# jcyk/gtos

Hardware: AMD Instinct MI355X
Metric: graphs/sec training step (100-node AMR, batch 64) (higher is better)
Workload: dtype bf16

## Files before the change

### gtos_amd/_lib.py

```python
import ctypes
import os
import threading

import torch

_HERE = os.path.dirname(os.path.abspath(__file__))
LIB_PATH = os.path.join(_HERE, "csrc", "libgtos_hip.so")
ABI_VERSION = 25

c_p, c_i, c_l, c_f, c_u64 = ctypes.c_void_p, ctypes.c_int, ctypes.c_int64, ctypes.c_float, ctypes.c_uint64

SIGNATURES = {
    "gtos_abi_version": [],
    "gtos_pathtrie_dev_workspace": [c_l, c_l, c_p],
    "gtos_pathtrie_dev_phase_a": [c_i, c_l, c_p, c_p, c_p, c_p, c_p, c_p, c_p, ctypes.c_size_t, c_p],
    "gtos_pathtrie_dev_phase_b": [c_l, c_l, c_i, c_i, c_i, c_i, c_p, c_p, c_p, c_p, c_p, ctypes.c_size_t, c_p],
    "gtos_relbatch_dev_workspace": [c_l, c_p],
    "gtos_relbatch_dev_phase_a": [c_p, c_p, c_p, ctypes.c_size_t, c_p],
    "gtos_relbatch_dev_phase_b": [c_p, c_l, c_p, c_p, ctypes.c_size_t, c_p],
    "gtos_relbatch_dev_all_count": [c_p, c_p, c_p, ctypes.c_size_t, c_p],
    "gtos_relbatch_dev_all_keys": [c_p, c_p, c_p, ctypes.c_size_t, c_p],
    "gtos_relbatch_dev_all_fill": [c_p, c_l, c_p, c_p, ctypes.c_size_t, c_p],
    "gtos_relindex_dev_workspace": [c_l, c_p],
    "gtos_relindex_dev_phase_a": [c_p, c_p, c_p, ctypes.c_size_t, c_p],
    "gtos_relindex_dev_phase_b": [c_p, c_l, c_p, c_p, ctypes.c_size_t, c_p],
    "gtos_gemm": [c_i, c_i, c_i, c_i, c_i, c_i, c_i, c_p, c_l, c_p, c_l, c_p, c_l, c_p, c_i, c_f, c_u64, c_i, c_i, c_p, c_l, c_p],
    "gtos_rel_attn_fwd": [c_i] * 7 + [c_p, c_l, c_p, c_l, c_p, c_l, c_p, c_p, c_p, c_p, c_f, c_f, c_u64, c_p, c_l, c_p, c_p, c_p],
    "gtos_rel_attn_bwd": [c_i] * 7 + [c_p, c_l, c_p, c_l, c_p, c_l, c_p, c_p, c_p, c_p, c_p, c_f, c_f, c_u64,
                                      c_p, c_l, c_p, c_p, c_p, c_l, c_p, c_p, c_l, c_p, c_l, c_p, c_l, c_p, c_l, c_p, c_p, c_p],
    "gtos_rel_attn_bwd_bank": [c_i] * 5 + [c_p, c_l, c_p, c_l, c_p, c_p, c_p, c_p, c_p, c_p, c_p, c_p, c_i, c_p, c_l, c_p, c_p],
    "gtos_ln_residual_fwd": [c_i, c_i, c_i, c_p, c_p, c_f, c_u64, c_p, c_p, c_f, c_p, c_p, c_p, c_p],
    "gtos_ln_residual_bwd": [c_i, c_i, c_i, c_p, c_p, c_p, c_f, c_u64, c_p, c_p, c_p, c_p, c_p, c_p, c_p, c_p],
    "gtos_ln_residual_fwd2": [c_i, c_i, c_i, c_i, c_i, c_p, c_p, c_f, c_u64, c_p, c_p, c_f, c_p, c_p, c_p, c_p, c_p],
    "gtos_ln_residual_bwd2": [c_i, c_i, c_i, c_i, c_i, c_p, c_p, c_p, c_p, c_f, c_u64, c_p, c_p, c_p, c_p, c_p, c_p, c_p, c_p],
    "gtos_relu_dropout_bwd": [c_i, c_l, c_p, c_p, c_f, c_p],
    "gtos_colsum": [c_i, c_i, c_i, c_l, c_p, c_p, c_p],
    "gtos_gru_cell_fwd": [c_i, c_i, c_i, c_p, c_p, c_p, c_p, c_l, c_p, c_p, c_f, c_u64, c_l, c_p],
    "gtos_gru_step_fwd": [c_i, c_i, c_p, c_l, c_i, c_p, c_p, c_p, c_p, c_p, c_p, c_p, c_p, c_p, c_p, c_p, c_p, c_i, c_p, c_l, c_p, c_p, c_p, c_l,
                          c_f, c_u64, c_l, c_p],
    "gtos_gru_step_bwd": [c_i, c_i, c_p, c_i, c_p, c_p, c_p, c_p, c_p, c_l, c_p, c_i, c_l, c_p, c_f, c_u64, c_l, c_p, c_i, c_p, c_p, c_p, c_i, c_p],
    "gtos_gru_step_bwd_fused": [c_i, c_i, c_p, c_i, c_p, c_p, c_p, c_p, c_p, c_l, c_p, c_i, c_l, c_p, c_f, c_u64, c_l, c_p, c_i, c_p, c_p, c_p, c_i,
                                c_p, c_p, c_l, c_i, c_i, c_f, c_u64, c_l, c_p],
    "gtos_gru_weight_grads": [c_i, c_i, c_i, c_i, c_p, c_p, c_l, c_p, c_l, c_p, c_l, c_p, c_l, c_p, c_l, c_p],
    "gtos_gemm_tn_batch": [c_i, c_p, c_p, c_p, c_p, c_p, c_p, c_p, c_p, c_p, c_p, c_p],
    "gtos_embed_packed_paths": [c_i, c_i, c_i, c_l, c_p, c_p, c_p, c_p, c_i, c_i, c_p, c_f, c_u64, c_p, c_i, c_p, c_p],
    "gtos_segment_sum_rows": [c_i, c_p, c_p, c_p, c_p, c_p, c_p, c_p, c_l, c_i, c_p, c_p, c_l, c_p, c_p, c_p],
    "gtos_segment_sum_stream": [c_i, c_i, c_p, c_p, c_p, c_p, c_p, c_p, c_i, c_p, c_l, c_i, c_p, c_l, c_p, c_p],
    "gtos_segment_sum_finish": [c_i, c_p, c_p, c_i, c_p, c_l, c_p],
    "gtos_segment_sum_ranges": [c_i, c_p, c_p, c_l, c_i, c_p, c_l, c_p],
    "gtos_gru_cell_bwd": [c_i, c_i, c_i, c_p, c_p, c_p, c_l, c_p, c_p, c_p, c_f, c_u64, c_l, c_p, c_i, c_p],
    "gtos_relation_gather_mean": [c_i, c_l, c_i, c_i, c_p, c_p, c_i, c_p, c_p],
    "gtos_embed_rows_fwd": [c_i, c_l, c_i, c_i, c_p, c_p, c_p, c_f, c_u64, c_p],
    "gtos_embed_rows_bwd": [c_i, c_l, c_i, c_i, c_i, c_p, c_p, c_p, c_f, c_u64, c_p, c_l, c_p],
    "gtos_copy_nll_fwd": [c_i, c_i, c_i, c_i, c_i, c_p, c_l, c_p, c_p, c_p, c_p, c_l, c_p, c_p, c_p, c_p],
    "gtos_copy_nll_bwd": [c_i, c_i, c_i, c_i, c_i, c_p, c_l, c_p, c_p, c_p, c_p, c_l, c_p, c_p, c_p, c_p, c_p, c_p, c_p],
    "gtos_copy_ll_fwd": [c_i, c_i, c_i, c_i, c_i, c_i, c_p, c_l, c_p, c_p, c_p, c_p, c_p],
    "gtos_copy_nll_ls_prep": [c_i, c_i, c_i, c_p, c_p, c_l, c_p],
    "gtos_copy_nll_ls_fwd": [c_i] * 5 + [c_p, c_l, c_p, c_p, c_p, c_l, c_f, c_p, c_l, c_p, c_p, c_p, c_p],
    "gtos_copy_nll_ls_bwd": [c_i] * 5 + [c_p, c_l, c_p, c_p, c_p, c_l, c_f, c_p, c_l, c_p, c_p, c_p, c_p, c_p, c_p, c_p],
    "gtos_copy_eval_fwd": [c_i, c_i, c_i, c_i, c_i, c_p, c_l, c_p, c_p, c_p, c_p, c_l, c_p, c_p, c_p, c_p],
    "gtos_eval_accumulate": [c_i, c_i, c_p, c_p, c_p, c_l, c_p, c_p, c_p, c_p, c_p],
    "gtos_beam_topk": [c_i, c_i, c_i, c_p, c_l, c_p, c_p, c_p],
    "gtos_beam_advance": [c_i] * 7 + [c_p] * 13,
    "gtos_beam_reorder": [c_i, c_p, c_p, c_l, c_i, c_i, c_i, c_i, c_p, c_p, c_p, c_p, c_i, c_i, c_p, c_p, c_p, c_p, c_i, c_l, c_p, c_p,
                          c_p, c_p],
    "gtos_sample_step": [c_i] * 7 + [c_f, c_i, c_f, c_u64, c_p, c_l] + [c_p] * 11 + [c_i, c_l] + [c_p] * 4,
    "gtos_highway_fwd": [c_i, c_l, c_i, c_p, c_p, c_p, c_p],
    "gtos_highway_bwd": [c_i, c_l, c_i, c_p, c_p, c_p, c_p, c_p, c_p],
    "gtos_max_relu_fwd": [c_i, c_l, c_i, c_i, c_p, c_p, c_p, c_p],
    "gtos_max_relu_bwd": [c_i, c_l, c_i, c_i, c_p, c_p, c_p, c_p, c_p],
    "gtos_token_row_fwd": [c_i, c_l, c_i, c_i, c_i, c_p, c_p, c_p, c_p, c_f, c_u64, c_p],
    "gtos_token_row_bwd": [c_i, c_l, c_i, c_i, c_i, c_p, c_p, c_p, c_p, c_f, c_u64, c_p],
    "gtos_sqnorm": [c_l, c_p, c_p, c_p],
    "gtos_adam_step": [c_l, c_p, c_p, c_p, c_p, c_f, c_f, c_f, c_f, c_f, c_f, c_p, c_f, c_p, c_p],
    "gtos_cast_f32_to_bf16": [c_l, c_p, c_p, c_p],
    "gtos_transpose_batch_bf16": [c_i, c_p, c_p, c_i, c_p, c_p, c_p],
    "gtos_step_control": [c_i, c_p, c_p, c_p, c_i, c_i, c_p, c_p],
    "gtos_set_seed_epoch": [c_p],
    "gtos_adam_step_ctl": [c_l, c_p, c_p, c_p, c_p, c_p, c_f, c_f, c_f, c_f, c_f, c_p, c_f, c_p, c_p],
}

_lib = None
_load_lock = threading.Lock()


class GtosHipError(RuntimeError):
    pass


def load():
    global _lib
    if _lib is not None:
        return _lib
    with _load_lock:
        if _lib is not None:
            return _lib
        if not os.path.exists(LIB_PATH):
            raise GtosHipError("%s is missing: run `python -m gtos_amd.build` (or __graft_entry__.build()); "
                               "there is no CPU fallback for the gtos hot path" % LIB_PATH)
        lib = ctypes.CDLL(LIB_PATH)
        for name, args in SIGNATURES.items():
            fn = getattr(lib, name)
            fn.argtypes = args
            fn.restype = ctypes.c_int
        if lib.gtos_abi_version() != ABI_VERSION:
            raise GtosHipError("libgtos_hip.so ABI %d != binding ABI %d: rebuild" % (lib.gtos_abi_version(), ABI_VERSION))
        _lib = lib
    return _lib


def call(name, *args):
    rc = getattr(load(), name)(*args)
    if rc != 0:
        raise GtosHipError("%s failed with code %d (%s)" % (
            name, rc, "HIP launch error" if rc > 0 else "unsupported argument/shape"))


def ptr(t):
    return None if t is None else t.data_ptr()


_raw_stream = None


def stream():
    global _raw_stream
    if _raw_stream:
        return _raw_stream(torch.cuda.current_device())
    pub = torch.cuda.current_stream().cuda_stream
    if _raw_stream is None:
        try:
            raw = torch._C._cuda_getCurrentRawStream
            ok = raw(torch.cuda.current_device()) == pub
            probe = torch.cuda.Stream()
            with torch.cuda.stream(probe):
                ok = ok and raw(torch.cuda.current_device()) == probe.cuda_stream == torch.cuda.current_stream().cuda_stream
            ok = ok and raw(torch.cuda.current_device()) == pub
            _raw_stream = raw if ok else False
        except Exception:
            _raw_stream = False
    return pub


def dt(t):
    if t.dtype == torch.float32:
        return 0
    if t.dtype == torch.bfloat16:
        return 1
    raise GtosHipError("unsupported dtype %s" % t.dtype)


def require_cuda(*ts):
    for t in ts:
        if t is not None and not t.is_cuda:
            raise GtosHipError("gtos_amd ops run on the GPU only (got a %s tensor); there is no CPU fallback" % t.device)
```

### gtos_amd/csrc/gru_step.hip

```cpp
#include <cstdlib>
#include "common.h"

__attribute__((visibility("hidden"))) const void* gtos_zero_block();

#define GTOS_VMCNT(n) __builtin_amdgcn_s_waitcnt(0x0F70 | ((n) & 15) | (((n) >> 4) << 14))
#ifndef GTOS_RACE_DEMO
#define GTOS_VMCNT_LDS(n) __builtin_amdgcn_s_waitcnt(0x0070 | ((n) & 15) | (((n) >> 4) << 14))
#define GTOS_LGKM0() __builtin_amdgcn_s_waitcnt(0xc07f)
#else
#define GTOS_VMCNT_LDS(n) GTOS_VMCNT(n)
#define GTOS_LGKM0()
#endif

namespace {

constexpr int ROWB = 128, BK = 64, TM = 128, TC = 64, WROWS = 3 * TC;
constexpr int A_BYTES = TM * ROWB, B_BYTES = WROWS * ROWB;

__device__ __forceinline__ int swz(int row) { return ((row >> 1) & 7) ^ ((row >> 4) & 3); }
__device__ __forceinline__ int lds_off(int r, int c) { return r * ROWB + ((c ^ swz(r)) << 4); }

struct StepArgs {
    const bf16_t* x; int64_t ldx; int in_dim; const bf16_t* w_ih; const float* b_ih;
    const bf16_t* xg;
    const bf16_t* gf; const int* gf_idx; const bf16_t* gb; const int* gb_idx;
    const bf16_t* h_in; const int* h_idx; const bf16_t* w_hh; const float* b_hh;
    bf16_t* h_out; int n_out; bf16_t* h_fin; bf16_t* gates; bf16_t* y; int64_t ldy;
    int64_t ld_fin; const int* fin_idx;
    float p_drop; uint64_t seed; int64_t drop_base;
    int rows, hs; const void* zeros;
};

__device__ __forceinline__ void dma_rows(const bf16_t* __restrict__ base, const U128* __restrict__ zeros, int64_t ld, int rows_total,
                                         int row0, int k0, int kend, char* tile, int wave, int lane,
                                         const int* __restrict__ gather = nullptr) {
#pragma unroll
    for (int it = 0; it < TM / 32; ++it) {
        const int blk = it * 4 + wave, rl = blk * 8 + (lane >> 3);
        const int c = (lane & 7) ^ swz(rl);
        const int r = row0 + rl, k = k0 + c * 8;
        const bool ok = r < rows_total && k + 8 <= kend;
        const int64_t sr = (gather && ok) ? gather[r] : r;
        const void* src = ok ? static_cast<const void*>(base + sr * ld + k) : static_cast<const void*>(zeros);
        __builtin_amdgcn_global_load_lds((const __attribute__((address_space(1))) void*)src,
                                         (__attribute__((address_space(3))) void*)(tile + blk * 1024), 16, 0, 0);
    }
}

__device__ __forceinline__ void dma_weights(const bf16_t* __restrict__ w, const U128* __restrict__ zeros, int64_t ld, int hs,
                                            int c0, int k0, int kend, char* tile, int wave, int lane) {
#pragma unroll
    for (int it = 0; it < WROWS / 32; ++it) {
        const int blk = it * 4 + wave, rl = blk * 8 + (lane >> 3);
        const int g = rl >> 6, nt = (rl >> 4) & 3, q = (rl >> 2) & 3, e = rl & 3;
        const int wrow = g * hs + c0 + q * 16 + nt * 4 + e;
        const int c = (lane & 7) ^ swz(rl);
        const int k = k0 + c * 8;
        const bool ok = k + 8 <= kend;
        const void* src = ok ? static_cast<const void*>(w + (int64_t)wrow * ld + k) : static_cast<const void*>(zeros);
        __builtin_amdgcn_global_load_lds((const __attribute__((address_space(1))) void*)src,
                                         (__attribute__((address_space(3))) void*)(tile + blk * 1024), 16, 0, 0);
    }
}

struct RowSrc { const char* p[TM / 32]; int c[TM / 32]; };
__device__ __forceinline__ RowSrc row_src(const bf16_t* __restrict__ base, int64_t ld, int rows_total, int row0, int wave, int lane,
                                          const int* __restrict__ gather = nullptr, int zero_row = -1) {
    RowSrc s;
#pragma unroll
    for (int it = 0; it < TM / 32; ++it) {
        const int rl = (it * 4 + wave) * 8 + (lane >> 3);
        const int r = row0 + rl;
        s.c[it] = (lane & 7) ^ swz(rl);
        const bool ok = r < rows_total;
        const int64_t sr = (gather && ok) ? gather[r] : r;
        s.p[it] = (ok && sr != zero_row) ? reinterpret_cast<const char*>(base + sr * ld + s.c[it] * 8) : nullptr;
    }
    return s;
}
__device__ __forceinline__ void dma_rows_at(const RowSrc& s, const U128* __restrict__ zeros, int k0, int kend, char* tile, int wave) {
#pragma unroll
    for (int it = 0; it < TM / 32; ++it) {
        const bool ok = s.p[it] != nullptr && k0 + s.c[it] * 8 + 8 <= kend;
        const void* src = ok ? static_cast<const void*>(s.p[it] + (int64_t)k0 * 2) : static_cast<const void*>(zeros);
        __builtin_amdgcn_global_load_lds((const __attribute__((address_space(1))) void*)src,
                                         (__attribute__((address_space(3))) void*)(tile + (it * 4 + wave) * 1024), 16, 0, 0);
    }
}
__device__ __forceinline__ void dma_rows_at_z(const RowSrc& s, int k0, char* tile, int wave, int lane) {
#pragma unroll
    for (int it = 0; it < TM / 32; ++it) {
        char* blk = tile + (it * 4 + wave) * 1024;
        if (s.p[it] != nullptr)
            __builtin_amdgcn_global_load_lds((const __attribute__((address_space(1))) void*)(s.p[it] + (int64_t)k0 * 2),
                                             (__attribute__((address_space(3))) void*)blk, 16, 0, 0);
        else
            *reinterpret_cast<uint4*>(blk + lane * 16) = make_uint4(0, 0, 0, 0);
    }
}
struct WSrc { uint32_t off[WROWS / 32]; int c[WROWS / 32]; };
__device__ __forceinline__ WSrc w_src(int64_t ld, int hs, int c0, int wave, int lane) {
    WSrc s;
#pragma unroll
    for (int it = 0; it < WROWS / 32; ++it) {
        const int rl = (it * 4 + wave) * 8 + (lane >> 3);
        const int g = rl >> 6, nt = (rl >> 4) & 3, q = (rl >> 2) & 3, e = rl & 3;
        const int wrow = g * hs + c0 + q * 16 + nt * 4 + e;
        s.c[it] = (lane & 7) ^ swz(rl);
        s.off[it] = (uint32_t)(wrow * (int)ld + s.c[it] * 8) * 2u;
    }
    return s;
}
__device__ __forceinline__ void dma_weights_at(const WSrc& s, const bf16_t* __restrict__ w, const U128* __restrict__ zeros, int k0, int kend,
                                               char* tile, int wave) {
    const char* wk = reinterpret_cast<const char*>(w) + (int64_t)k0 * 2;
#pragma unroll
    for (int it = 0; it < WROWS / 32; ++it) {
        const bool ok = k0 + s.c[it] * 8 + 8 <= kend;
        const void* src = ok ? static_cast<const void*>(wk + s.off[it]) : static_cast<const void*>(zeros);
        __builtin_amdgcn_global_load_lds((const __attribute__((address_space(1))) void*)src,
                                         (__attribute__((address_space(3))) void*)(tile + (it * 4 + wave) * 1024), 16, 0, 0);
    }
}

template <int NG, int G2>
__device__ __forceinline__ void mma_tile(const char* As, const char* Bs, int wrow0, int fr, int fq, f32x4_t (&acc)[2][NG * 4]) {
#pragma unroll
    for (int ks = 0; ks < 2; ++ks) {
        bf16x8_t fa[2];
#pragma unroll
        for (int mt = 0; mt < 2; ++mt) fa[mt] = *reinterpret_cast<const bf16x8_t*>(As + lds_off(wrow0 + mt * 16 + fr, ks * 4 + fq));
#pragma unroll
        for (int g = 0; g < 3; ++g) {
            const int ag = g < 2 ? g : G2;
#pragma unroll
            for (int nt = 0; nt < 4; ++nt) {
                const bf16x8_t fb = *reinterpret_cast<const bf16x8_t*>(Bs + lds_off(g * 64 + nt * 16 + fr, ks * 4 + fq));
#pragma unroll
                for (int mt = 0; mt < 2; ++mt)
                    acc[mt][ag * 4 + nt] = __builtin_amdgcn_mfma_f32_16x16x32_bf16(fb, fa[mt], acc[mt][ag * 4 + nt], 0, 0, 0);
            }
        }
    }
}

__device__ __forceinline__ void ld16(const bf16_t* p, float (&v)[16]) {
    const uint4 a = *reinterpret_cast<const uint4*>(p), b = *reinterpret_cast<const uint4*>(p + 8);
    v[0] = lo_bf(a.x); v[1] = hi_bf(a.x); v[2] = lo_bf(a.y); v[3] = hi_bf(a.y);
    v[4] = lo_bf(a.z); v[5] = hi_bf(a.z); v[6] = lo_bf(a.w); v[7] = hi_bf(a.w);
    v[8] = lo_bf(b.x); v[9] = hi_bf(b.x); v[10] = lo_bf(b.y); v[11] = hi_bf(b.y);
    v[12] = lo_bf(b.z); v[13] = hi_bf(b.z); v[14] = lo_bf(b.w); v[15] = hi_bf(b.w);
}
__device__ __forceinline__ void st16(bf16_t* p, const float (&v)[16]) {
    *reinterpret_cast<uint4*>(p) = make_uint4(pack_bf(v[0], v[1]), pack_bf(v[2], v[3]), pack_bf(v[4], v[5]), pack_bf(v[6], v[7]));
    *reinterpret_cast<uint4*>(p + 8) = make_uint4(pack_bf(v[8], v[9]), pack_bf(v[10], v[11]), pack_bf(v[12], v[13]), pack_bf(v[14], v[15]));
}
__device__ __forceinline__ void ldf16(const float* p, float (&v)[16]) {
#pragma unroll
    for (int i = 0; i < 4; ++i) {
        const float4 a = *reinterpret_cast<const float4*>(p + i * 4);
        v[i * 4] = a.x; v[i * 4 + 1] = a.y; v[i * 4 + 2] = a.z; v[i * 4 + 3] = a.w;
    }
}

__device__ __forceinline__ float fast_tanh(float x) {
    const float e = __expf(2.f * x);
    return 1.f - 2.f * __builtin_amdgcn_rcpf(e + 1.f);
}

template <int MODE>
__device__ __forceinline__ void step_cell(const StepArgs& a, f32x4_t (&acc)[2][(MODE == 1 ? 4 : 3) * 4], int m0, int c0, int wave, int fr, int fq) {
    constexpr bool HAS_X = MODE == 1;
    constexpr int GH = HAS_X ? 3 : 2;
    const int cb = c0 + fq * 16, hs = a.hs;
    float bhr[16], bhz[16], bhn[16];
    ldf16(a.b_hh + cb, bhr); ldf16(a.b_hh + hs + cb, bhz); ldf16(a.b_hh + 2 * hs + cb, bhn);
    if constexpr (MODE != 0) {
        float t[16];
        ldf16(a.b_ih + cb, t);
#pragma unroll
        for (int i = 0; i < 16; ++i) bhr[i] += t[i];
        ldf16(a.b_ih + hs + cb, t);
#pragma unroll
        for (int i = 0; i < 16; ++i) bhz[i] += t[i];
    }
    const float ks = a.p_drop > 0.f ? 1.f / (1.f - a.p_drop) : 1.f;
#pragma unroll
    for (int mt = 0; mt < 2; ++mt) {
        const int m = m0 + wave * 32 + mt * 16 + fr;
        if (m >= a.rows) continue;
        float xr[16], xz[16], xn[16], hp[16];
        if constexpr (HAS_X) {
            ldf16(a.b_ih + 2 * hs + cb, xn);
#pragma unroll
            for (int i = 0; i < 16; ++i) { xr[i] = 0.f; xz[i] = 0.f; xn[i] += acc[mt][8 + (i >> 2)][i & 3]; }
        } else if constexpr (MODE == 2) {
            const bf16_t* fp = a.gf + (int64_t)a.gf_idx[m] * 3 * hs + cb;
            const bf16_t* bp = a.gb + (int64_t)a.gb_idx[m] * 3 * hs + cb;
            float t[16];
            ld16(fp, xr); ld16(bp, t);
#pragma unroll
            for (int i = 0; i < 16; ++i) xr[i] += t[i];
            ld16(fp + hs, xz); ld16(bp + hs, t);
#pragma unroll
            for (int i = 0; i < 16; ++i) xz[i] += t[i];
            ld16(fp + 2 * hs, xn); ld16(bp + 2 * hs, t);
#pragma unroll
            for (int i = 0; i < 16; ++i) xn[i] += t[i];
            ldf16(a.b_ih + 2 * hs + cb, t);
#pragma unroll
            for (int i = 0; i < 16; ++i) xn[i] += t[i];
        } else {
            const bf16_t* xp = a.xg + (int64_t)m * 3 * hs + cb;
            ld16(xp, xr); ld16(xp + hs, xz); ld16(xp + 2 * hs, xn);
        }
        ld16(a.h_in + (int64_t)(a.h_idx ? a.h_idx[m] : m) * hs + cb, hp);
        float gr[16], gz[16], gn[16], hn[16], o[16];
#pragma unroll
        for (int i = 0; i < 16; ++i) {
            gr[i] = 1.f / (1.f + __expf(-(xr[i] + acc[mt][(i >> 2)][i & 3] + bhr[i])));
            gz[i] = 1.f / (1.f + __expf(-(xz[i] + acc[mt][4 + (i >> 2)][i & 3] + bhz[i])));
            hn[i] = acc[mt][GH * 4 + (i >> 2)][i & 3] + bhn[i];
            hn[i] = bf2f(f2bf(hn[i]));
            gn[i] = fast_tanh(xn[i] + gr[i] * hn[i]);
            o[i] = (1.f - gz[i]) * gn[i] + gz[i] * hp[i];
        }
        bf16_t* gp = a.gates + (int64_t)m * 4 * hs + cb;
        st16(gp, gr); st16(gp + hs, gz); st16(gp + 2 * hs, gn);
        st16(gp + 3 * hs, hn);
        bf16_t* hdst = m < a.n_out ? a.h_out + (int64_t)m * hs + cb
                                   : a.h_fin + (int64_t)(a.fin_idx ? a.fin_idx[m] : m) * a.ld_fin + cb;
        st16(hdst, o);
        if (a.y) {
            if (a.p_drop > 0.f) {
#pragma unroll
                for (int i = 0; i < 16; ++i)
                    o[i] = drop_keep(a.seed, (uint64_t)(a.drop_base + (int64_t)m * a.ldy + cb + i), a.p_drop) ? o[i] * ks : 0.f;
            }
            st16(a.y + (int64_t)m * a.ldy + cb, o);
        }
    }
}

template <int MODE>
__global__ __launch_bounds__(256, 2) void gru_step_fwd_kernel(StepArgs a) {
    if (a.p_drop > 0.f) a.seed = live_seed(a.seed);
    constexpr bool HAS_X = MODE == 1;
    constexpr int NG = HAS_X ? 4 : 3;
    constexpr int GH = HAS_X ? 3 : 2;
    __shared__ __attribute__((aligned(16))) char lds[A_BYTES + B_BYTES];
    char* As = lds;
    char* Bs = lds + A_BYTES;
    const int lane = threadIdx.x & 63, wave = __builtin_amdgcn_readfirstlane(threadIdx.x >> 6);
    const int fr = lane & 15, fq = lane >> 4;
    const int nC = a.hs / TC;
    const int xcd = blockIdx.x & 7, sq = blockIdx.x >> 3;
    const int m0 = ((sq / nC) * 8 + xcd) * TM, c0 = (sq % nC) * TC;
    if (m0 >= a.rows) return;
    const U128* Z = static_cast<const U128*>(a.zeros);

    f32x4_t acc[2][NG * 4];
#pragma unroll
    for (int i = 0; i < 2; ++i)
#pragma unroll
        for (int j = 0; j < NG * 4; ++j) acc[i][j] = f32x4_t{0.f, 0.f, 0.f, 0.f};

    if constexpr (HAS_X) {
        const RowSrc xs = row_src(a.x, a.ldx, a.rows, m0, wave, lane);
        const WSrc ws = w_src(a.in_dim, a.hs, c0, wave, lane);
        for (int k0 = 0; k0 < a.in_dim; k0 += BK) {
            dma_rows_at(xs, Z, k0, a.in_dim, As, wave);
            dma_weights_at(ws, a.w_ih, Z, k0, a.in_dim, Bs, wave);
            __syncthreads();
            mma_tile<NG, 2>(As, Bs, wave * 32, fr, fq, acc);
            __syncthreads();
        }
    }
    {
        const RowSrc hsrc = row_src(a.h_in, a.hs, a.rows, m0, wave, lane, a.h_idx);
        const WSrc ws = w_src(a.hs, a.hs, c0, wave, lane);
        for (int k0 = 0; k0 < a.hs; k0 += BK) {
            dma_rows_at(hsrc, Z, k0, a.hs, As, wave);
            dma_weights_at(ws, a.w_hh, Z, k0, a.hs, Bs, wave);
            __syncthreads();
            mma_tile<NG, GH>(As, Bs, wave * 32, fr, fq, acc);
            __syncthreads();
        }
    }

    step_cell<MODE>(a, acc, m0, c0, wave, fr, fq);
}


__global__ __launch_bounds__(512, 2) void gru_step_fwd_a2w3_kernel(StepArgs a) {
    constexpr int TMW = 256, AW = TMW * ROWB;
    if (a.p_drop > 0.f) a.seed = live_seed(a.seed);
    __shared__ __attribute__((aligned(16))) char sa0[AW];
    __shared__ __attribute__((aligned(16))) char sa1[AW];
    __shared__ __attribute__((aligned(16))) char sw0[B_BYTES];
    __shared__ __attribute__((aligned(16))) char sw1[B_BYTES];
    __shared__ __attribute__((aligned(16))) char sa2[AW];
    const int lane = threadIdx.x & 63, wave = __builtin_amdgcn_readfirstlane(threadIdx.x >> 6);
    const int fr = lane & 15, fq = lane >> 4;
    const int hs = a.hs, nC = hs / TC;
    const int xcd = blockIdx.x & 7, sq = blockIdx.x >> 3;
    const int m0 = ((sq / nC) * 8 + xcd) * TMW, c0 = (sq % nC) * TC;
    if (m0 >= a.rows) return;
    const int nkx = a.in_dim / BK, nk = nkx + hs / BK;
    uint32_t axo[4], aho[4], bxo[3], bho[3];
#pragma unroll
    for (int i = 0; i < 4; ++i) {
        const int rl = (i * 8 + wave) * 8 + (lane >> 3);
        const int r = min(m0 + rl, a.rows - 1) - m0;
        const uint32_t c = (uint32_t)(((lane & 7) ^ swz(rl)) << 4);
        axo[i] = (uint32_t)r * (uint32_t)(a.ldx * 2) + c;
        aho[i] = (uint32_t)r * (uint32_t)(hs * 2) + c;
    }
#pragma unroll
    for (int i = 0; i < 3; ++i) {
        const int rl = (i * 8 + wave) * 8 + (lane >> 3);
        const int g = rl >> 6, nt = (rl >> 4) & 3, q = (rl >> 2) & 3, e = rl & 3;
        const int wrow = g * hs + c0 + q * 16 + nt * 4 + e;
        const uint32_t c = (uint32_t)(((lane & 7) ^ swz(rl)) << 4);
        bxo[i] = (uint32_t)wrow * (uint32_t)(a.in_dim * 2) + c;
        bho[i] = (uint32_t)wrow * (uint32_t)(hs * 2) + c;
    }
    const char* Xb = reinterpret_cast<const char*>(a.x + (int64_t)m0 * a.ldx);
    const char* Hb = reinterpret_cast<const char*>(a.h_in + (int64_t)m0 * hs);
    const char* Wi = reinterpret_cast<const char*>(a.w_ih);
    const char* Wh = reinterpret_cast<const char*>(a.w_hh);

    f32x4_t acc[2][16];
#pragma unroll
    for (int i = 0; i < 2; ++i)
#pragma unroll
        for (int j = 0; j < 16; ++j) acc[i][j] = f32x4_t{0.f, 0.f, 0.f, 0.f};

#define GTOS_DMA1(src, dst)                                                                                                   \
    __builtin_amdgcn_global_load_lds((const __attribute__((address_space(1))) void*)(src),                                    \
                                     (__attribute__((address_space(3))) void*)(dst), 16, 0, 0)
#define GTOS_A2W3_DMA_A(slot, s_)                                                                                             \
    {                                                                                                                         \
        const int st_ = min((s_), nk - 1);                                                                                    \
        const bool px_ = st_ < nkx;                                                                                           \
        const char* ab_ = px_ ? Xb + st_ * ROWB : Hb + (st_ - nkx) * ROWB;                                                    \
        GTOS_DMA1(ab_ + (px_ ? axo[0] : aho[0]), (slot) + (0 * 8 + wave) * 1024);                                             \
        GTOS_DMA1(ab_ + (px_ ? axo[1] : aho[1]), (slot) + (1 * 8 + wave) * 1024);                                             \
        GTOS_DMA1(ab_ + (px_ ? axo[2] : aho[2]), (slot) + (2 * 8 + wave) * 1024);                                             \
        GTOS_DMA1(ab_ + (px_ ? axo[3] : aho[3]), (slot) + (3 * 8 + wave) * 1024);                                             \
    }
#define GTOS_A2W3_DMA_W(slot, s_)                                                                                             \
    {                                                                                                                         \
        const int st_ = min((s_), nk - 1);                                                                                    \
        const bool px_ = st_ < nkx;                                                                                           \
        const char* bb_ = px_ ? Wi + st_ * ROWB : Wh + (st_ - nkx) * ROWB;                                                    \
        GTOS_DMA1(bb_ + (px_ ? bxo[0] : bho[0]), (slot) + (0 * 8 + wave) * 1024);                                             \
        GTOS_DMA1(bb_ + (px_ ? bxo[1] : bho[1]), (slot) + (1 * 8 + wave) * 1024);                                             \
        GTOS_DMA1(bb_ + (px_ ? bxo[2] : bho[2]), (slot) + (2 * 8 + wave) * 1024);                                             \
    }
#define GTOS_A2W3_STEP(sa_, sw_, sa_n, sw_n, s_)                                                                              \
    {                                                                                                                         \
        GTOS_VMCNT_LDS(4);                                  \
        __builtin_amdgcn_s_barrier();                       \
        GTOS_A2W3_DMA_W(sw_n, (s_) + 1);                                                                                      \
        GTOS_A2W3_DMA_A(sa_n, (s_) + 2);                                                                                      \
        {                                                                                                                     \
            _Pragma("unroll") for (int ks = 0; ks < 2; ++ks) {                                                                \
                bf16x8_t fa[2], fb[12];                                                                                       \
                _Pragma("unroll") for (int mt = 0; mt < 2; ++mt)                                                              \
                    fa[mt] = *reinterpret_cast<const bf16x8_t*>((sa_) + lds_off(wave * 32 + mt * 16 + fr, ks * 4 + fq));      \
                _Pragma("unroll") for (int t = 0; t < 12; ++t)                                                                \
                    fb[t] = *reinterpret_cast<const bf16x8_t*>((sw_) + lds_off(t * 16 + fr, ks * 4 + fq));                    \
                _Pragma("unroll") for (int g = 0; g < 2; ++g)                                                                 \
                    _Pragma("unroll") for (int nt = 0; nt < 4; ++nt)                                                          \
                        _Pragma("unroll") for (int mt = 0; mt < 2; ++mt)                                                      \
                            acc[mt][g * 4 + nt] = __builtin_amdgcn_mfma_f32_16x16x32_bf16(fb[g * 4 + nt], fa[mt], acc[mt][g * 4 + nt], 0, 0, 0); \
                if ((s_) < nkx) {                                                                                             \
                    _Pragma("unroll") for (int nt = 0; nt < 4; ++nt)                                                          \
                        _Pragma("unroll") for (int mt = 0; mt < 2; ++mt)                                                      \
                            acc[mt][8 + nt] = __builtin_amdgcn_mfma_f32_16x16x32_bf16(fb[8 + nt], fa[mt], acc[mt][8 + nt], 0, 0, 0); \
                } else {                                                                                                      \
                    _Pragma("unroll") for (int nt = 0; nt < 4; ++nt)                                                          \
                        _Pragma("unroll") for (int mt = 0; mt < 2; ++mt)                                                      \
                            acc[mt][12 + nt] = __builtin_amdgcn_mfma_f32_16x16x32_bf16(fb[8 + nt], fa[mt], acc[mt][12 + nt], 0, 0, 0); \
                }                                                                                                             \
            }                                                                                                                 \
        }                                                                                                                     \
    }

    if (nk > 0) {
        GTOS_A2W3_DMA_A(sa0, 0);
        GTOS_A2W3_DMA_W(sw0, 0);
        GTOS_A2W3_DMA_A(sa1, 1);
    }
    for (int s = 0; s + 6 <= nk; s += 6) {
        GTOS_A2W3_STEP(sa0, sw0, sa2, sw1, s);
        GTOS_A2W3_STEP(sa1, sw1, sa0, sw0, s + 1);
        GTOS_A2W3_STEP(sa2, sw0, sa1, sw1, s + 2);
        GTOS_A2W3_STEP(sa0, sw1, sa2, sw0, s + 3);
        GTOS_A2W3_STEP(sa1, sw0, sa0, sw1, s + 4);
        GTOS_A2W3_STEP(sa2, sw1, sa1, sw0, s + 5);
    }
    GTOS_VMCNT(0);
#undef GTOS_A2W3_STEP
#undef GTOS_A2W3_DMA_W
#undef GTOS_A2W3_DMA_A
#undef GTOS_DMA1
    step_cell<1>(a, acc, m0, c0, wave, fr, fq);
}


struct Raw16 { uint4 a, b; };
__device__ __forceinline__ void unpack16(const Raw16& r, float (&v)[16]) {
    v[0] = lo_bf(r.a.x); v[1] = hi_bf(r.a.x); v[2] = lo_bf(r.a.y); v[3] = hi_bf(r.a.y);
    v[4] = lo_bf(r.a.z); v[5] = hi_bf(r.a.z); v[6] = lo_bf(r.a.w); v[7] = hi_bf(r.a.w);
    v[8] = lo_bf(r.b.x); v[9] = hi_bf(r.b.x); v[10] = lo_bf(r.b.y); v[11] = hi_bf(r.b.y);
    v[12] = lo_bf(r.b.z); v[13] = hi_bf(r.b.z); v[14] = lo_bf(r.b.w); v[15] = hi_bf(r.b.w);
}
__device__ __forceinline__ Raw16 ldraw16(const bf16_t* p) {
    Raw16 r;
    r.a = *reinterpret_cast<const uint4*>(p);
    r.b = *reinterpret_cast<const uint4*>(p + 8);
    return r;
}

constexpr int P_ROWS = 32;
constexpr int P_TM = 4 * P_ROWS;

template <int KT>
__global__ __launch_bounds__(256, 1) void gru_l1_fwd_persistent_kernel(StepArgs a, int n_workers) {
    extern __shared__ __attribute__((aligned(16))) char plds[];
    constexpr int HS = 64 * KT;
    constexpr int A_TILE = P_ROWS * ROWB;
    const int lane = threadIdx.x & 63, wave = __builtin_amdgcn_readfirstlane(threadIdx.x >> 6);
    const int fr = lane & 15, fq = lane >> 4;
    char* Ws = plds;
    char* Aw = plds + KT * B_BYTES + wave * (KT * A_TILE);
    const int nC = KT;
    const int xcd = blockIdx.x & 7, sub = blockIdx.x >> 3;
    const int ct = sub % nC, worker = (sub / nC) * 8 + xcd, c0 = ct * TC;
    const U128* Z = static_cast<const U128*>(a.zeros);
#pragma unroll
    for (int kt = 0; kt < KT; ++kt) dma_weights(a.w_hh, Z, HS, HS, c0, kt * BK, HS, Ws + kt * B_BYTES, wave, lane);
    __syncthreads();

    const int cb = c0 + fq * 16;
    float bhr[16], bhz[16], bhn[16], bin[16];
    {
        float t[16];
        ldf16(a.b_hh + cb, bhr); ldf16(a.b_ih + cb, t);
#pragma unroll
        for (int i = 0; i < 16; ++i) bhr[i] += t[i];
        ldf16(a.b_hh + HS + cb, bhz); ldf16(a.b_ih + HS + cb, t);
#pragma unroll
        for (int i = 0; i < 16; ++i) bhz[i] += t[i];
        ldf16(a.b_hh + 2 * HS + cb, bhn); ldf16(a.b_ih + 2 * HS + cb, bin);
    }
    const int n_tiles = (a.rows + P_TM - 1) / P_TM;

    auto dma_A = [&](int tile) {
        const int r0 = tile * P_TM + wave * P_ROWS;
#pragma unroll
        for (int kt = 0; kt < KT; ++kt)
#pragma unroll
            for (int it = 0; it < P_ROWS / 8; ++it) {
                const int rl = it * 8 + (lane >> 3);
                const int c = (lane & 7) ^ swz(rl);
                const int r = r0 + rl;
                const void* src = r < a.rows ? static_cast<const void*>(a.h_in + (int64_t)r * HS + kt * BK + c * 8)
                                             : static_cast<const void*>(Z);
                __builtin_amdgcn_global_load_lds((const __attribute__((address_space(1))) void*)src,
                                                 (__attribute__((address_space(3))) void*)(Aw + kt * A_TILE + it * 1024), 16, 0, 0);
            }
    };
    struct Pre { Raw16 f[3], b[3], h; };
    auto gather = [&](int tile, Pre (&P)[2]) {
#pragma unroll
        for (int mt = 0; mt < 2; ++mt) {
            int m = tile * P_TM + wave * P_ROWS + mt * 16 + fr;
            m = m < a.rows ? m : a.rows - 1;
            const bf16_t* fp = a.gf + (int64_t)a.gf_idx[m] * 3 * HS + cb;
            const bf16_t* bp = a.gb + (int64_t)a.gb_idx[m] * 3 * HS + cb;
#pragma unroll
            for (int g = 0; g < 3; ++g) { P[mt].f[g] = ldraw16(fp + g * HS); P[mt].b[g] = ldraw16(bp + g * HS); }
            P[mt].h = ldraw16(a.h_in + (int64_t)m * HS + cb);
        }
    };

    int tile = worker;
    Pre P[2];
    if (tile < n_tiles) { dma_A(tile); gather(tile, P); }
    for (; tile < n_tiles; tile += n_workers) {
        f32x4_t acc[2][12];
#pragma unroll
        for (int i = 0; i < 2; ++i)
#pragma unroll
            for (int j = 0; j < 12; ++j) acc[i][j] = f32x4_t{0.f, 0.f, 0.f, 0.f};
#pragma unroll
        for (int kt = 0; kt < KT; ++kt) {
            const char* As = Aw + kt * A_TILE;
            const char* Bs = Ws + kt * B_BYTES;
#pragma unroll
            for (int ks = 0; ks < 2; ++ks) {
                bf16x8_t fa[2];
#pragma unroll
                for (int mt = 0; mt < 2; ++mt) fa[mt] = *reinterpret_cast<const bf16x8_t*>(As + lds_off(mt * 16 + fr, ks * 4 + fq));
#pragma unroll
                for (int g = 0; g < 3; ++g)
#pragma unroll
                    for (int nt = 0; nt < 4; ++nt) {
                        const bf16x8_t fb = *reinterpret_cast<const bf16x8_t*>(Bs + lds_off(g * 64 + nt * 16 + fr, ks * 4 + fq));
#pragma unroll
                        for (int mt = 0; mt < 2; ++mt)
                            acc[mt][g * 4 + nt] = __builtin_amdgcn_mfma_f32_16x16x32_bf16(fb, fa[mt], acc[mt][g * 4 + nt], 0, 0, 0);
                    }
            }
        }
        __builtin_amdgcn_s_waitcnt(0xc07f);
        const int next = tile + n_workers;
        if (next < n_tiles) dma_A(next);
#pragma unroll
        for (int mt = 0; mt < 2; ++mt) {
            const int m = tile * P_TM + wave * P_ROWS + mt * 16 + fr;
            float xr[16], xz[16], xn[16], hp[16], t[16];
            unpack16(P[mt].f[0], xr); unpack16(P[mt].b[0], t);
#pragma unroll
            for (int i = 0; i < 16; ++i) xr[i] += t[i];
            unpack16(P[mt].f[1], xz); unpack16(P[mt].b[1], t);
#pragma unroll
            for (int i = 0; i < 16; ++i) xz[i] += t[i];
            unpack16(P[mt].f[2], xn); unpack16(P[mt].b[2], t);
#pragma unroll
            for (int i = 0; i < 16; ++i) xn[i] += t[i] + bin[i];
            unpack16(P[mt].h, hp);
            float gr[16], gz[16], gn[16], hn[16], o[16];
#pragma unroll
            for (int i = 0; i < 16; ++i) {
                gr[i] = 1.f / (1.f + __expf(-(xr[i] + acc[mt][(i >> 2)][i & 3] + bhr[i])));
                gz[i] = 1.f / (1.f + __expf(-(xz[i] + acc[mt][4 + (i >> 2)][i & 3] + bhz[i])));
                hn[i] = bf2f(f2bf(acc[mt][8 + (i >> 2)][i & 3] + bhn[i]));
                gn[i] = fast_tanh(xn[i] + gr[i] * hn[i]);
                o[i] = (1.f - gz[i]) * gn[i] + gz[i] * hp[i];
            }
            if (m < a.rows) {
                bf16_t* gp = a.gates + (int64_t)m * 4 * HS + cb;
                st16(gp, gr); st16(gp + HS, gz); st16(gp + 2 * HS, gn);
                st16(gp + 3 * HS, hn);
                bf16_t* hdst = m < a.n_out ? a.h_out + (int64_t)m * HS + cb
                                           : a.h_fin + (int64_t)(a.fin_idx ? a.fin_idx[m] : m) * a.ld_fin + cb;
                st16(hdst, o);
            }
        }
        if (next < n_tiles) gather(next, P);
    }
}


struct StepBwdArgs {
    const bf16_t* d4_prev; int rows_prev; const bf16_t* wh_t;
    const bf16_t* gates; const bf16_t* hprev; const int* hprev_idx; const bf16_t* dy; int64_t ldy;
    void* dh; int dh_bf16; int64_t ld_dh; bf16_t* d4; float* bias_part; int n_partials;
    bf16_t* hp_out;
    const int* sum_idx;
    const void* dh_src;
    int zero_row;
    float p_drop; uint64_t seed; int64_t drop_base;
    int rows, hs; const void* zeros;
    const bf16_t* wi_t; bf16_t* dinp; int64_t ld_dinp; int n_in; int dinp_acc;
    float p_in; uint64_t seed_in; int64_t in_drop_base;
};

#define GTOS_DPP(v, ctrl) __builtin_bit_cast(float, __builtin_amdgcn_update_dpp(0, __builtin_bit_cast(int, (v)), (ctrl), 0xF, 0xF, true))
__device__ __forceinline__ float row16_sum(float v) {
    v += GTOS_DPP(v, 0xB1); v += GTOS_DPP(v, 0x4E); v += GTOS_DPP(v, 0x141); v += GTOS_DPP(v, 0x140);
    return v;
}

__device__ __forceinline__ void dma_wt(const bf16_t* __restrict__ w, int64_t ld, int c0, int k0, char* tile, int wave, int lane) {
#pragma unroll
    for (int it = 0; it < TC / 32; ++it) {
        const int blk = it * 4 + wave, rl = blk * 8 + (lane >> 3);
        const int nt = (rl >> 4) & 3, q = (rl >> 2) & 3, e = rl & 3;
        const int wrow = c0 + q * 16 + nt * 4 + e;
        const int c = (lane & 7) ^ swz(rl);
        const void* src = static_cast<const void*>(w + (int64_t)wrow * ld + k0 + c * 8);
        __builtin_amdgcn_global_load_lds((const __attribute__((address_space(1))) void*)src,
                                         (__attribute__((address_space(3))) void*)(tile + blk * 1024), 16, 0, 0);
    }
}

template <int NB, bool SKIP>
__device__ __forceinline__ void kloop_a2(const bf16_t* __restrict__ A, int64_t lda, int rows_total, int m0, const bf16_t* __restrict__ W,
                                         int64_t ldw, int n0, int nsub, int hs, const U128* __restrict__ Z, char* a0, char* a1, char* ws,
                                         f32x4_t (&acc)[2][NB * 4], int wave, int lane) {
    const int fr = lane & 15, fq = lane >> 4, nst = 3 * hs / BK;
#define GTOS_KA_A(slot, s_)                                                                                                   \
    {                                                                                                                         \
        const int kk_ = min((s_), nst - 1) * BK, ak_ = SKIP ? (kk_ < 2 * hs ? kk_ : kk_ + hs) : kk_;                            \
        dma_rows(A, Z, lda, rows_total, m0, ak_, ak_ + BK, (slot), wave, lane);                                               \
    }
#define GTOS_KA_STEP(cur, nxt, s_)                                                                                            \
    {                                                                                                                         \
        _Pragma("unroll") for (int h = 0; h < NB; ++h)                                                                        \
            if (h < nsub) dma_wt(W, ldw, n0 + h * TC, (s_) * BK, ws + h * TC * ROWB, wave, lane);                             \
        GTOS_VMCNT_LDS(0);                                                                                                    \
        __builtin_amdgcn_s_barrier();                                          \
        GTOS_KA_A(nxt, (s_) + 1);                                                                                             \
        __builtin_amdgcn_sched_barrier(0);                                                                                    \
        _Pragma("unroll") for (int ks = 0; ks < 2; ++ks) {                                                                    \
            bf16x8_t fa[2], fb[4];                                                                                            \
            _Pragma("unroll") for (int mt = 0; mt < 2; ++mt)                                                                  \
                fa[mt] = *reinterpret_cast<const bf16x8_t*>((cur) + lds_off(wave * 32 + mt * 16 + fr, ks * 4 + fq));          \
            _Pragma("unroll") for (int h = 0; h < NB; ++h) {                                                                  \
                if (h < nsub) {                                                                                               \
                    _Pragma("unroll") for (int nt = 0; nt < 4; ++nt)                                                          \
                        fb[nt] = *reinterpret_cast<const bf16x8_t*>(ws + h * TC * ROWB + lds_off(nt * 16 + fr, ks * 4 + fq)); \
                    _Pragma("unroll") for (int mt = 0; mt < 2; ++mt)                                                          \
                        _Pragma("unroll") for (int nt = 0; nt < 4; ++nt)                                                      \
                            acc[mt][h * 4 + nt] = __builtin_amdgcn_mfma_f32_16x16x32_bf16(fb[nt], fa[mt], acc[mt][h * 4 + nt], 0, 0, 0); \
                }                                                                                                             \
            }                                                                                                                 \
        }                                                                                                                     \
        GTOS_LGKM0();                                       \
        __builtin_amdgcn_s_barrier();                               \
    }
    GTOS_KA_A(a0, 0);
    int s = 0;
    for (; s + 2 <= nst; s += 2) {
        GTOS_KA_STEP(a0, a1, s);
        GTOS_KA_STEP(a1, a0, s + 1);
    }
    if (s < nst) GTOS_KA_STEP(a0, a1, s);
    GTOS_VMCNT(0);
    __builtin_amdgcn_s_barrier();
#undef GTOS_KA_STEP
#undef GTOS_KA_A
}

template <int NS>
__device__ __forceinline__ void dinp_tile(const StepBwdArgs& a, int m0, int n0, char* As, char* Bs, char* A1, int wave, int lane) {
    if (m0 >= a.rows_prev) return;
    const int fr = lane & 15, fq = lane >> 4, hs = a.hs;
    const U128* Z = static_cast<const U128*>(a.zeros);
    const int nsub = min(NS, (a.n_in - n0) / TC);
    f32x4_t acc[2][NS * 4];
#pragma unroll
    for (int i = 0; i < 2; ++i)
#pragma unroll
        for (int j = 0; j < NS * 4; ++j) acc[i][j] = f32x4_t{0.f, 0.f, 0.f, 0.f};
    kloop_a2<NS, false>(a.d4_prev, 4 * (int64_t)hs, a.rows_prev, m0, a.wi_t, 3 * (int64_t)hs, n0, nsub, hs, Z, As, A1, Bs, acc, wave, lane);
    const float ks_in = a.p_in > 0.f ? 1.f / (1.f - a.p_in) : 1.f;
    const uint64_t seed_in = a.p_in > 0.f ? live_seed(a.seed_in) : 0;
    Raw16 oldv[2][NS];
    if (a.dinp_acc) {
#pragma unroll
        for (int mt = 0; mt < 2; ++mt) {
            const int m = min(m0 + wave * 32 + mt * 16 + fr, a.rows_prev - 1);
#pragma unroll
            for (int h = 0; h < NS; ++h)
                if (h < nsub) oldv[mt][h] = ldraw16(a.dinp + (int64_t)m * a.ld_dinp + n0 + h * TC + fq * 16);
        }
    }
#pragma unroll
    for (int mt = 0; mt < 2; ++mt) {
        const int m = m0 + wave * 32 + mt * 16 + fr;
        if (m >= a.rows_prev) continue;
#pragma unroll
        for (int h = 0; h < NS; ++h) {
            if (h >= nsub) continue;
            const int nb = n0 + h * TC + fq * 16;
            float v[16];
#pragma unroll
            for (int i = 0; i < 16; ++i) v[i] = acc[mt][h * 4 + (i >> 2)][i & 3];
            if (a.p_in > 0.f) {
#pragma unroll
                for (int i = 0; i < 16; ++i)
                    v[i] = drop_keep(seed_in, (uint64_t)(a.in_drop_base + (int64_t)m * a.n_in + nb + i), a.p_in) ? v[i] * ks_in : 0.f;
            }
            bf16_t* dp = a.dinp + (int64_t)m * a.ld_dinp + nb;
            if (a.dinp_acc) {
                float old[16];
                unpack16(oldv[mt][h], old);
#pragma unroll
                for (int i = 0; i < 16; ++i) v[i] += old[i];
            }
            st16(dp, v);
        }
    }
}

template <int NS = 2>
__global__ __launch_bounds__(256, 3) void gru_step_bwd_kernel(StepBwdArgs a) {
    if (a.p_drop > 0.f) a.seed = live_seed(a.seed);
    __shared__ __attribute__((aligned(16))) char lds[A_BYTES];
    __shared__ __attribute__((aligned(16))) char lds_w[NS * TC * ROWB];
    __shared__ __attribute__((aligned(16))) char lds_a1[A_BYTES];
    __shared__ float btab[4 * TC];
    char* As = lds;
    char* Bs = lds_w;
    const int lane = threadIdx.x & 63, wave = __builtin_amdgcn_readfirstlane(threadIdx.x >> 6);
    const int fr = lane & 15, fq = lane >> 4;
    const int hs = a.hs, nC = hs / TC;
    const int nB = a.dinp ? (a.n_in + NS * TC - 1) / (NS * TC) : 0, per = nC + nB;
    const int xcd = blockIdx.x & 7, sq = blockIdx.x >> 3;
    const int m0 = ((sq / per) * 8 + xcd) * TM, role = sq % per;
    if (role >= nC) { dinp_tile<NS>(a, m0, (role - nC) * NS * TC, As, Bs, lds_a1, wave, lane); return; }
    const int c0 = role * TC;
    if (m0 >= a.rows) return;
    const U128* Z = static_cast<const U128*>(a.zeros);
    if (a.bias_part) { btab[threadIdx.x] = 0.f; }

    f32x4_t acc[2][4];
#pragma unroll
    for (int i = 0; i < 2; ++i)
#pragma unroll
        for (int j = 0; j < 4; ++j) acc[i][j] = f32x4_t{0.f, 0.f, 0.f, 0.f};

    if (a.d4_prev && a.sum_idx) {
        const RowSrc src = row_src(a.d4_prev, 4 * (int64_t)hs, a.rows, m0, wave, lane, a.sum_idx, a.zero_row);
        for (int kk = 0; kk < 3 * hs; kk += BK) {
            const int ak = kk < 2 * hs ? kk : kk + hs;
            dma_rows_at_z(src, ak, As, wave, lane);
            dma_wt(a.wh_t, 3 * (int64_t)hs, c0, kk, Bs, wave, lane);
            __syncthreads();
#pragma unroll
            for (int ks = 0; ks < 2; ++ks) {
                bf16x8_t fa[2], fb[4];
#pragma unroll
                for (int mt = 0; mt < 2; ++mt) fa[mt] = *reinterpret_cast<const bf16x8_t*>(As + lds_off(wave * 32 + mt * 16 + fr, ks * 4 + fq));
#pragma unroll
                for (int nt = 0; nt < 4; ++nt) fb[nt] = *reinterpret_cast<const bf16x8_t*>(Bs + lds_off(nt * 16 + fr, ks * 4 + fq));
#pragma unroll
                for (int mt = 0; mt < 2; ++mt)
#pragma unroll
                    for (int nt = 0; nt < 4; ++nt)
                        acc[mt][nt] = __builtin_amdgcn_mfma_f32_16x16x32_bf16(fb[nt], fa[mt], acc[mt][nt], 0, 0, 0);
            }
            __syncthreads();
        }
    } else if (a.d4_prev && m0 < a.rows_prev) {
        kloop_a2<1, true>(a.d4_prev, 4 * (int64_t)hs, a.rows_prev, m0, a.wh_t, 3 * (int64_t)hs, c0, 1, hs, Z, As, lds_a1, Bs, acc, wave, lane);
    } else if (a.bias_part) {
        __syncthreads();
    }

    const int cb = c0 + fq * 16;
    const float ks = a.p_drop > 0.f ? 1.f / (1.f - a.p_drop) : 1.f;
#pragma unroll
    for (int mt = 0; mt < 2; ++mt) {
        const int m_raw = m0 + wave * 32 + mt * 16 + fr;
        const bool valid = m_raw < a.rows;
        const int m = valid ? m_raw : a.rows - 1;
        float gr[16], gz[16], gn[16], hn[16], hp[16], g[16];
        const bf16_t* gp = a.gates + (int64_t)m * 4 * hs + cb;
        ld16(gp, gr); ld16(gp + hs, gz); ld16(gp + 2 * hs, gn);
        ld16(gp + 3 * hs, hn);
        ld16(a.hprev + (int64_t)(a.hprev_idx ? a.hprev_idx[m] : m) * hs + cb, hp);
        float* dhp = static_cast<float*>(a.dh) + (int64_t)m * a.ld_dh + cb;
        bf16_t* dhb = static_cast<bf16_t*>(a.dh) + (int64_t)m * a.ld_dh + cb;
        if (a.sum_idx) {
            const int64_t sr = a.sum_idx[m];
            if (sr == a.zero_row) {
#pragma unroll
                for (int i = 0; i < 16; ++i) g[i] = 0.f;
            } else if (a.dh_bf16) ld16(static_cast<const bf16_t*>(a.dh_src) + sr * hs + cb, g);
            else ldf16(static_cast<const float*>(a.dh_src) + sr * hs + cb, g);
        } else if (a.dh_bf16) ld16(dhb, g); else ldf16(dhp, g);
#pragma unroll
        for (int i = 0; i < 16; ++i) g[i] += acc[mt][i >> 2][i & 3];
        if (a.dy) {
            float dyv[16];
            ld16(a.dy + (int64_t)m * a.ldy + cb, dyv);
#pragma unroll
            for (int i = 0; i < 16; ++i) {
                float t2 = dyv[i];
                if (a.p_drop > 0.f) t2 = drop_keep(a.seed, (uint64_t)(a.drop_base + (int64_t)m * a.ldy + cb + i), a.p_drop) ? t2 * ks : 0.f;
                g[i] += t2;
            }
        }
        float dr_[16], dz_[16], dn_[16], dhn[16];
#pragma unroll
        for (int i = 0; i < 16; ++i) {
            const float dn = g[i] * (1.f - gz[i]);
            const float dz = g[i] * (hp[i] - gn[i]);
            dn_[i] = dn * (1.f - gn[i] * gn[i]);
            dhn[i] = dn_[i] * gr[i];
            dr_[i] = dn_[i] * hn[i] * gr[i] * (1.f - gr[i]);
            dz_[i] = dz * gz[i] * (1.f - gz[i]);
            g[i] *= gz[i];
            if (!valid) { dn_[i] = 0.f; dhn[i] = 0.f; dr_[i] = 0.f; dz_[i] = 0.f; }
        }
        if (valid) {
            if (a.dh_bf16) {
                st16(dhb, g);
            } else {
#pragma unroll
                for (int i = 0; i < 4; ++i)
                    *reinterpret_cast<float4*>(dhp + i * 4) = make_float4(g[i * 4], g[i * 4 + 1], g[i * 4 + 2], g[i * 4 + 3]);
            }
            bf16_t* dp = a.d4 + (int64_t)m * 4 * hs + cb;
            st16(dp, dr_); st16(dp + hs, dz_); st16(dp + 2 * hs, dn_); st16(dp + 3 * hs, dhn);
            if (a.hp_out) st16(a.hp_out + (int64_t)m * hs + cb, hp);
        }
        if (a.bias_part) {
#pragma unroll
            for (int i = 0; i < 16; ++i) {
                const float t0 = row16_sum(bf2f(f2bf(dr_[i]))), t1 = row16_sum(bf2f(f2bf(dz_[i])));
                const float t2 = row16_sum(bf2f(f2bf(dn_[i]))), t3 = row16_sum(bf2f(f2bf(dhn[i])));
                if (fr == 0) {
                    atomicAdd(&btab[0 * TC + fq * 16 + i], t0); atomicAdd(&btab[1 * TC + fq * 16 + i], t1);
                    atomicAdd(&btab[2 * TC + fq * 16 + i], t2); atomicAdd(&btab[3 * TC + fq * 16 + i], t3);
                }
            }
        }
    }
    if (a.bias_part) {
        __syncthreads();
        const int q = threadIdx.x >> 6, ch = threadIdx.x & 63;
        float* dst = a.bias_part + (int64_t)(blockIdx.x % a.n_partials) * 4 * hs + q * hs + c0 + ch;
        atomicAdd(dst, btab[threadIdx.x]);
    }
}


}

extern "C" int gtos_gru_step_fwd(int rows, int hs, const void* x, int64_t ldx, int in_dim, const void* w_ih, const float* b_ih,
                                 const void* xg, const void* gf, const int* gf_idx, const void* gb, const int* gb_idx,
                                 const void* h_in, const int* h_idx, const void* w_hh, const float* b_hh,
                                 void* h_out, int n_out, void* h_fin, int64_t ld_fin, const int* fin_idx, void* gates, void* y, int64_t ldy,
                                 float p_drop, uint64_t seed, int64_t drop_base, void* stream) {
    if (rows <= 0) return 0;
    if (hs <= 0 || hs % TC) return -22;
    if (!h_in || !w_hh || !b_hh || !gates) return -23;
    if ((n_out > 0 && !h_out) || (n_out < rows && !h_fin)) return -23;
    if (h_fin && (ld_fin < hs || ld_fin % 8)) return -25;
    const int mode = x ? 1 : (gf ? 2 : 0);
    if (mode == 1) {
        if (!w_ih || !b_ih || in_dim <= 0 || in_dim % 8 || ldx % 8 || (uintptr_t)x % 16 || (uintptr_t)w_ih % 16) return -24;
    } else if (mode == 2) {
        if (!gb || !gf_idx || !gb_idx || !b_ih || (uintptr_t)gf % 16 || (uintptr_t)gb % 16) return -24;
    } else if (!xg || (uintptr_t)xg % 16) return -24;
    if ((uintptr_t)h_in % 16 || (uintptr_t)w_hh % 16 || (uintptr_t)gates % 16 || (uintptr_t)h_out % 16 || (uintptr_t)h_fin % 16 ||
        (uintptr_t)b_hh % 16 || (uintptr_t)b_ih % 16) return -25;
    if (y && ((uintptr_t)y % 16 || ldy % 8)) return -25;
    StepArgs a;
    a.x = (const bf16_t*)x; a.ldx = ldx; a.in_dim = in_dim; a.w_ih = (const bf16_t*)w_ih; a.b_ih = b_ih; a.xg = (const bf16_t*)xg;
    a.gf = (const bf16_t*)gf; a.gf_idx = gf_idx; a.gb = (const bf16_t*)gb; a.gb_idx = gb_idx;
    a.h_in = (const bf16_t*)h_in; a.h_idx = h_idx; a.w_hh = (const bf16_t*)w_hh; a.b_hh = b_hh;
    a.h_out = (bf16_t*)h_out; a.n_out = n_out; a.h_fin = (bf16_t*)h_fin; a.gates = (bf16_t*)gates; a.y = (bf16_t*)y; a.ldy = ldy;
    a.ld_fin = ld_fin; a.fin_idx = fin_idx;
    a.p_drop = p_drop; a.seed = seed; a.drop_base = drop_base; a.rows = rows; a.hs = hs;
    a.zeros = gtos_zero_block();
    if (!a.zeros) return -5;
    const long long nM = (rows + TM - 1) / TM, nC = hs / TC;
    const long long nblk = ((nM + 7) / 8) * 8 * nC;
    if (nblk > 0x7fffffffLL) return -6;
    hipStream_t s = static_cast<hipStream_t>(stream);
    if (mode == 2 && hs == 256 && !h_idx && !y && rows >= 16384) {
        constexpr int KT = 4;
        const size_t lds_bytes = (size_t)KT * B_BYTES + 4 * KT * P_ROWS * ROWB;
        static bool configured = false;
        if (!configured) {
            if (hipFuncSetAttribute(reinterpret_cast<const void*>(gru_l1_fwd_persistent_kernel<KT>),
                                    hipFuncAttributeMaxDynamicSharedMemorySize, (int)lds_bytes) != hipSuccess) return -7;
            configured = true;
        }
        const int n_cu = 256, n_workers = n_cu / KT;
        hipLaunchKernelGGL(gru_l1_fwd_persistent_kernel<KT>, dim3(n_cu), dim3(256), lds_bytes, s, a, n_workers);
        GTOS_CHECK_LAUNCH();
        return 0;
    }
    static const bool use_a2w3 = !(getenv("GTOS_GRU_FWD_A2W3") && getenv("GTOS_GRU_FWD_A2W3")[0] == '0');
    if (mode == 1 && use_a2w3 && rows >= 8192 && in_dim % 64 == 0 && (in_dim / 64 + hs / 64) % 6 == 0 && !h_idx && ldx < (1 << 20) &&
        (int64_t)3 * hs * (in_dim > hs ? in_dim : hs) * 2 < (1LL << 31)) {
        const long long nM8 = (rows + 255) / 256, nblk8 = ((nM8 + 7) / 8) * 8 * nC;
        hipLaunchKernelGGL(gru_step_fwd_a2w3_kernel, dim3((unsigned)nblk8), dim3(512), 0, s, a);
    }
    else if (mode == 1) hipLaunchKernelGGL(gru_step_fwd_kernel<1>, dim3((unsigned)nblk), dim3(256), 0, s, a);
    else if (mode == 2) hipLaunchKernelGGL(gru_step_fwd_kernel<2>, dim3((unsigned)nblk), dim3(256), 0, s, a);
    else hipLaunchKernelGGL(gru_step_fwd_kernel<0>, dim3((unsigned)nblk), dim3(256), 0, s, a);
    GTOS_CHECK_LAUNCH();
    return 0;
}

extern "C" int gtos_gru_step_bwd_fused(int rows, int hs, const void* d4_prev, int rows_prev, const void* w_hh_t,
                                       const void* gates, const void* hprev, const int* hprev_idx, const void* dy, int64_t ldy,
                                       void* dh, int dh_dtype, int64_t ld_dh, void* d4, float p_drop, uint64_t seed, int64_t drop_base,
                                       float* bias_partials, int n_partials, void* hprev_out, const int* sum_idx, const void* dh_src,
                                       int zero_row,
                                       const void* w_ih_t, void* dinp, int64_t ld_dinp, int n_in, int dinp_accumulate, float p_in,
                                       uint64_t seed_in, int64_t in_drop_base, void* stream) {
    const bool role_b = dinp != nullptr && d4_prev != nullptr && rows_prev > 0;
    if (rows <= 0 && !role_b) return 0;
    if (hs <= 0 || hs % TC) return -22;
    if (rows > 0) {
        if (!gates || !hprev || !dh || !d4 || (d4_prev && !w_hh_t)) return -23;
        if (sum_idx && (!dh_src || (uintptr_t)dh_src % 16)) return -23;
    }
    if (dinp && (!d4_prev || !w_ih_t || sum_idx)) return -23;
    if (dinp && (n_in <= 0 || n_in % TC || ld_dinp < n_in || ld_dinp % 8 || (uintptr_t)dinp % 16 || (uintptr_t)w_ih_t % 16)) return -27;
    if (bias_partials && n_partials < 1) return -26;
    if ((uintptr_t)d4_prev % 16 || (uintptr_t)w_hh_t % 16 || (uintptr_t)gates % 16 || (uintptr_t)hprev % 16 || (uintptr_t)dh % 16 ||
        (uintptr_t)d4 % 16 || (dy && ((uintptr_t)dy % 16 || ldy % 8)) || (rows > 0 && (ld_dh < hs || ld_dh % 8)) ||
        (uintptr_t)hprev_out % 16) return -25;
    StepBwdArgs a;
    a.d4_prev = (const bf16_t*)d4_prev; a.rows_prev = d4_prev ? rows_prev : 0; a.wh_t = (const bf16_t*)w_hh_t;
    a.gates = (const bf16_t*)gates; a.hprev = (const bf16_t*)hprev; a.hprev_idx = hprev_idx; a.dy = (const bf16_t*)dy; a.ldy = ldy;
    a.dh = dh; a.dh_bf16 = dh_dtype == GTOS_BF16; a.ld_dh = ld_dh; a.d4 = (bf16_t*)d4; a.bias_part = bias_partials; a.n_partials = n_partials;
    a.hp_out = (bf16_t*)hprev_out; a.sum_idx = sum_idx; a.dh_src = dh_src; a.zero_row = sum_idx ? zero_row : -1;
    a.wi_t = (const bf16_t*)w_ih_t; a.dinp = role_b ? (bf16_t*)dinp : nullptr; a.ld_dinp = ld_dinp; a.n_in = n_in; a.dinp_acc = dinp_accumulate;
    a.p_in = p_in; a.seed_in = seed_in; a.in_drop_base = in_drop_base;
    a.p_drop = p_drop; a.seed = seed; a.drop_base = drop_base; a.rows = rows > 0 ? rows : 0; a.hs = hs;
    a.zeros = gtos_zero_block();
    if (!a.zeros) return -5;
    const long long cover = role_b && rows_prev > a.rows ? rows_prev : a.rows;
    const long long nM = (cover + TM - 1) / TM, per = hs / TC + (role_b ? (n_in + 2 * TC - 1) / (2 * TC) : 0);
    const long long nblk = ((nM + 7) / 8) * 8 * per;
    if (nblk > 0x7fffffffLL) return -6;
    hipLaunchKernelGGL(gru_step_bwd_kernel<2>, dim3((unsigned)nblk), dim3(256), 0, static_cast<hipStream_t>(stream), a);
    GTOS_CHECK_LAUNCH();
    return 0;
}

extern "C" int gtos_gru_step_bwd(int rows, int hs, const void* d4_prev, int rows_prev, const void* w_hh_t,
                                 const void* gates, const void* hprev, const int* hprev_idx, const void* dy, int64_t ldy, void* dh, int dh_dtype,
                                 int64_t ld_dh, void* d4, float p_drop, uint64_t seed, int64_t drop_base, float* bias_partials,
                                 int n_partials, void* hprev_out, const int* sum_idx, const void* dh_src, int zero_row, void* stream) {
    return gtos_gru_step_bwd_fused(rows, hs, d4_prev, rows_prev, w_hh_t, gates, hprev, hprev_idx, dy, ldy, dh, dh_dtype, ld_dh, d4,
                                   p_drop, seed, drop_base, bias_partials, n_partials, hprev_out, sum_idx, dh_src, zero_row,
                                   nullptr, nullptr, 0, 0, 0, 0.f, 0, 0, stream);
}

GTOS_SEED_EPOCH_SETTER(gru_step)
```

### gtos_amd/csrc/rowops.hip

```cpp
#include "common.h"

namespace {

constexpr int LN_MAXC = 2;

template <typename TX, typename TR, typename TY>
__global__ __launch_bounds__(256) void ln_fwd_kernel(int rows, int d, const TX* __restrict__ x, const TR* __restrict__ r,
                                                     float p_drop, uint64_t seed, const float* __restrict__ gamma,
                                                     const float* __restrict__ beta, float eps, TY* __restrict__ y, bf16_t* __restrict__ y2,
                                                     float* __restrict__ mean, float* __restrict__ rstd) {
    if (p_drop > 0.f) seed = live_seed(seed);
    const int lane = threadIdx.x & 63;
    const int row = blockIdx.x * 4 + (threadIdx.x >> 6);
    if (row >= rows) return;
    const float ks = p_drop > 0.f ? 1.f / (1.f - p_drop) : 1.f;
    float z[LN_MAXC][8];
    float s = 0.f;
#pragma unroll
    for (int cI = 0; cI < LN_MAXC; ++cI) {
        const int c = (cI * 64 + lane) * 8;
#pragma unroll
        for (int e = 0; e < 8; ++e) z[cI][e] = 0.f;
        if (c < d) {
            Vec8<TX>::load(x + (int64_t)row * d + c, z[cI]);
// ... 816 lines not shown
                                    void* stream) {
    return gtos_ln_residual_fwd2(dtype, dtype, dtype, rows, d, x, r, p_drop, seed, gamma, beta, eps, y, nullptr, mean, rstd, stream);
}

extern "C" int gtos_ln_residual_bwd2(int x_dtype, int r_dtype, int y_dtype, int rows, int d, const void* dy, const void* dy2_bf16,
                                     const void* x, const void* r, float p_drop, uint64_t seed, const float* gamma, const float* mean,
                                     const float* rstd, void* dx, void* dr, float* dgamma, float* dbeta, void* stream) {
    if (d % 8 || d > 512 * LN_MAXC) return -20;
    if (rows <= 0) return 0;
    if (!dy && !dy2_bf16) return -23;
    if ((uintptr_t)x % 16 || (uintptr_t)r % 16 || (uintptr_t)dy % 16 || (uintptr_t)dy2_bf16 % 16 || (uintptr_t)dx % 16 || (uintptr_t)dr % 16) return -25;
    hipStream_t s = static_cast<hipStream_t>(stream);
    int nb = (rows + 31) / 32; if (nb > 256) nb = 256; if (nb < 1) nb = 1;
    dim3 grid(nb), block(256);
#define X(dx_, dr_, dy_, TX, TR, TY)                                                                                                   \
    if (x_dtype == dx_ && r_dtype == dr_ && y_dtype == dy_) {                                                                          \
        hipLaunchKernelGGL((ln_bwd_kernel<TX, TR, TY>), grid, block, 0, s, rows, d, (const TY*)dy, (const bf16_t*)dy2_bf16,            \
                           (const TX*)x, (const TR*)r, p_drop, seed, gamma, mean, rstd, (TX*)dx, (TR*)dr, dgamma, dbeta);              \
        GTOS_CHECK_LAUNCH();                                                                                                           \
        return 0;                                                                                                                      \
    }
    GTOS_LN_COMBOS(X)
#undef X
    return -21;
}

extern "C" int gtos_ln_residual_bwd(int dtype, int rows, int d, const void* dy, const void* x, const void* r, float p_drop,
                                    uint64_t seed, const float* gamma, const float* mean, const float* rstd,
                                    void* dx, void* dr, float* dgamma, float* dbeta, void* stream) {
    return gtos_ln_residual_bwd2(dtype, dtype, dtype, rows, d, dy, nullptr, x, r, p_drop, seed, gamma, mean, rstd, dx, dr, dgamma, dbeta,
                                 stream);
}

extern "C" int gtos_relu_dropout_bwd(int dtype, int64_t n, void* dh, const void* h, float p_drop, void* stream) {
    if (n % 8) return -21;
    if (n == 0) return 0;
    hipStream_t s = static_cast<hipStream_t>(stream);
    const float ks = p_drop > 0.f ? 1.f / (1.f - p_drop) : 1.f;
    dim3 grid(grid_for(n / 8, 256)), block(256);
    if (dtype == GTOS_BF16) hipLaunchKernelGGL(relu_drop_bwd_kernel<bf16_t>, grid, block, 0, s, n / 8, (bf16_t*)dh, (const bf16_t*)h, ks);
    else hipLaunchKernelGGL(relu_drop_bwd_kernel<float>, grid, block, 0, s, n / 8, (float*)dh, (const float*)h, ks);
    GTOS_CHECK_LAUNCH();
    return 0;
}

extern "C" int gtos_colsum(int dtype, int rows, int N, int64_t ld, const void* dy, float* out, void* stream) {
    if (rows <= 0 || N <= 0) return 0;
    hipStream_t s = static_cast<hipStream_t>(stream);
    const int gx = (N + 511) / 512;
    int rpb = (rows + 1023) / 1024; if (rpb < 64) rpb = 64;
    dim3 grid(gx, (rows + rpb - 1) / rpb), block(256);
    if (dtype == GTOS_BF16) hipLaunchKernelGGL(colsum_kernel<bf16_t>, grid, block, 0, s, rows, N, ld, (const bf16_t*)dy, out, rpb);
    else hipLaunchKernelGGL(colsum_kernel<float>, grid, block, 0, s, rows, N, ld, (const float*)dy, out, rpb);
    GTOS_CHECK_LAUNCH();
    return 0;
}

extern "C" int gtos_gru_cell_fwd(int dtype, int rows, int hs, const void* xg, const void* hg, void* h, void* y, int64_t ldy,
                                 void* hprev_save, void* gates, float p_drop, uint64_t seed, int64_t drop_base, void* stream) {
    if (hs % 8) return -22;
    if (rows <= 0) return 0;
    hipStream_t s = static_cast<hipStream_t>(stream);
    dim3 grid(grid_for((int64_t)rows * hs / 8, 256)), block(256);
    if (dtype == GTOS_BF16) hipLaunchKernelGGL(gru_fwd_kernel<bf16_t>, grid, block, 0, s, rows, hs, (const bf16_t*)xg, (const bf16_t*)hg, (bf16_t*)h, (bf16_t*)y, ldy, (bf16_t*)hprev_save, (bf16_t*)gates, p_drop, seed, drop_base);
    else hipLaunchKernelGGL(gru_fwd_kernel<float>, grid, block, 0, s, rows, hs, (const float*)xg, (const float*)hg, (float*)h, (float*)y, ldy, (float*)hprev_save, (float*)gates, p_drop, seed, drop_base);
    GTOS_CHECK_LAUNCH();
    return 0;
}

extern "C" int gtos_gru_cell_bwd(int dtype, int rows, int hs, const void* gates, const void* hprev, const void* dy, int64_t ldy,
                                 float* dh, void* dxg, void* dhg, float p_drop, uint64_t seed, int64_t drop_base,
                                 float* bias_partials, int n_partials, void* stream) {
    if (hs % 8) return -22;
    if (rows <= 0) return 0;
    if (bias_partials && (256 % (hs / 8) != 0 || n_partials < 1)) return -26;
    hipStream_t s = static_cast<hipStream_t>(stream);
    int nb = grid_for((int64_t)rows * hs / 8, 256);
    if (bias_partials && nb > n_partials) nb = n_partials;
    dim3 grid(nb), block(256);
    const size_t sh = bias_partials ? (size_t)4 * hs * sizeof(float) : 0;
    if (dtype == GTOS_BF16) hipLaunchKernelGGL(gru_bwd_kernel<bf16_t>, grid, block, sh, s, rows, hs, (const bf16_t*)gates, (const bf16_t*)hprev, (const bf16_t*)dy, ldy, dh, (bf16_t*)dxg, (bf16_t*)dhg, p_drop, seed, drop_base, bias_partials);
    else hipLaunchKernelGGL(gru_bwd_kernel<float>, grid, block, sh, s, rows, hs, (const float*)gates, (const float*)hprev, (const float*)dy, ldy, dh, (float*)dxg, (float*)dhg, p_drop, seed, drop_base, bias_partials);
    GTOS_CHECK_LAUNCH();
    return 0;
}

extern "C" int gtos_relation_gather_mean(int dtype, int64_t P, int K, int d, const void* bank, const int64_t* idx, int zero_row0,
                                         void* out, void* stream) {
    if (d % 8) return -23;
    if (P <= 0) return 0;
    hipStream_t s = static_cast<hipStream_t>(stream);
    dim3 grid(grid_for(P * (d / 8), 256)), block(256);
    if (dtype == GTOS_BF16) hipLaunchKernelGGL(gather_mean_kernel<bf16_t>, grid, block, 0, s, P, K, d, (const bf16_t*)bank, idx, zero_row0, (bf16_t*)out);
    else hipLaunchKernelGGL(gather_mean_kernel<float>, grid, block, 0, s, P, K, d, (const float*)bank, idx, zero_row0, (float*)out);
    GTOS_CHECK_LAUNCH();
    return 0;
}


extern "C" int gtos_embed_rows_fwd(int dtype, int64_t n, int dim, int dim_pad, const int64_t* tok, const float* table, void* out,
                                   float p_drop, uint64_t seed, void* stream) {
    if (dim_pad % 8 || dim_pad < dim) return -24;
    if (n <= 0) return 0;
    hipStream_t s = static_cast<hipStream_t>(stream);
    dim3 grid(grid_for(n * (dim_pad / 8), 256)), block(256);
    if (dtype == GTOS_BF16) hipLaunchKernelGGL(embed_rows_fwd_kernel<bf16_t>, grid, block, 0, s, n, dim, dim_pad, tok, table, (bf16_t*)out, p_drop, seed);
    else hipLaunchKernelGGL(embed_rows_fwd_kernel<float>, grid, block, 0, s, n, dim, dim_pad, tok, table, (float*)out, p_drop, seed);
    GTOS_CHECK_LAUNCH();
    return 0;
}

extern "C" int gtos_embed_packed_paths(int dtype, int L, int R, int64_t n_rows, const int64_t* bank, const int* order, const int* offs,
                                       const float* table, int dim, int dim_pad, void* x, float p_drop, uint64_t seed, void* onehot, int vp,
                                       int64_t* tokens, void* stream) {
    if (dim_pad % 8 || dim_pad < dim || L < 1 || L > 64 || R < 1) return -24;
    if (onehot && (vp < 8 || vp % 8 || (uintptr_t)onehot % 16)) return -24;
    if (!bank || !order || !offs || !table || !x || (uintptr_t)x % 16) return -23;
    if (n_rows <= 0) return 0;
    hipStream_t s = static_cast<hipStream_t>(stream);
    dim3 grid(grid_for(n_rows * (dim_pad / 8), 256)), block(256);
    if (dtype == GTOS_BF16)
        hipLaunchKernelGGL(embed_packed_paths_kernel<bf16_t>, grid, block, 0, s, L, R, n_rows, bank, order, offs, table, dim, dim_pad, (bf16_t*)x,
                           p_drop, seed, (bf16_t*)onehot, vp, tokens);
    else
        hipLaunchKernelGGL(embed_packed_paths_kernel<float>, grid, block, 0, s, L, R, n_rows, bank, order, offs, table, dim, dim_pad, (float*)x,
                           p_drop, seed, (bf16_t*)onehot, vp, tokens);
    GTOS_CHECK_LAUNCH();
    return 0;
}

extern "C" int gtos_embed_rows_bwd(int dtype, int64_t n, int V, int dim, int dim_pad, const int64_t* tok, const void* dout,
                                   float* dtable, float p_drop, uint64_t seed, float* workspace, int64_t workspace_bytes, void* stream) {
    if (dim_pad % 8 || dim_pad < dim) return -24;
    const int use_lds = (size_t)V * dim_pad * 4 <= 60 * 1024;
    if (n <= 0) return 0;
    hipStream_t s = static_cast<hipStream_t>(stream);
    int64_t nb = (n + 511) / 512; if (nb > 2048) nb = 2048; if (nb < 1) nb = 1;
    const int64_t table_bytes = (int64_t)V * dim_pad * 4;
    float* partials = nullptr;
    if (use_lds && workspace && nb > 8) {
        if (workspace_bytes < table_bytes) return -24;
        const int64_t fit = workspace_bytes / table_bytes;
        if (nb > fit) nb = fit;
        partials = workspace;
    }
    const int64_t rpb = (n + nb - 1) / nb;
    dim3 grid((unsigned)((n + rpb - 1) / rpb)), block(256);
    const size_t sh = use_lds ? (size_t)table_bytes : 0;
#define GTOS_EMB_BWD(T, L) hipLaunchKernelGGL((embed_rows_bwd_kernel<T, L>), grid, block, sh, s, n, V, dim, dim_pad, tok, (const T*)dout, dtable, p_drop, seed, rpb, partials)
    if (dtype == GTOS_BF16) { if (use_lds) GTOS_EMB_BWD(bf16_t, true); else GTOS_EMB_BWD(bf16_t, false); }
    else { if (use_lds) GTOS_EMB_BWD(float, true); else GTOS_EMB_BWD(float, false); }
#undef GTOS_EMB_BWD
    GTOS_CHECK_LAUNCH();
    if (partials) {
        const int total = V * dim_pad;
        const int slices = grid.x >= 64 ? 16 : 1;
        hipLaunchKernelGGL(embed_reduce_kernel, dim3((total + 255) / 256, slices), dim3(256), 0, s, (int)grid.x, V, dim, dim_pad, partials, dtable);
        GTOS_CHECK_LAUNCH();
    }
    return 0;
}

extern "C" int gtos_segment_sum_rows(int n_chunks, const int* rows, const int* chunk_node, const int* chunk_start, const int* chunk_cnt,
                                     const int* chunk_slot, const void* src, const void* src2, int64_t ld_src, int width,
                                     void* dst, void* dst2, int64_t ld_dst, float* heavy, float* heavy2, void* stream) {
    if (n_chunks <= 0) return 0;
    if (width <= 0 || width % 8 || width > 1536 || ld_src % 8 || ld_dst % 8 || (uintptr_t)src % 16 || (uintptr_t)dst % 16 ||
        (uintptr_t)src2 % 16 || (uintptr_t)dst2 % 16) return -24;
    if (!chunk_node || !chunk_start || !chunk_cnt || !src || !dst || (chunk_slot && !heavy)) return -23;
    if (src2 && (!dst2 || (chunk_slot && !heavy2))) return -23;
    hipStream_t s = static_cast<hipStream_t>(stream);
    const int nblk = (n_chunks + 3) / 4;
    const dim3 grid((unsigned)(nblk < 4096 ? nblk : 4096)), block(256);
#define GTOS_SEG(S, Q) hipLaunchKernelGGL((seg_sum_kernel<S, Q>), grid, block, 0, s, n_chunks, rows, chunk_node, chunk_start, chunk_cnt, \
                                          chunk_slot, (const bf16_t*)src, (const bf16_t*)src2, ld_src, width, (bf16_t*)dst, (bf16_t*)dst2, \
                                          ld_dst, heavy, heavy2)
    if (src2) { if (width <= 512) GTOS_SEG(1, 2); else if (width <= 1024) GTOS_SEG(2, 2); else GTOS_SEG(3, 2); }
    else { if (width <= 512) GTOS_SEG(1, 1); else if (width <= 1024) GTOS_SEG(2, 1); else GTOS_SEG(3, 1); }
#undef GTOS_SEG
    GTOS_CHECK_LAUNCH();
    return 0;
}

extern "C" int gtos_segment_sum_stream(int n_chunks, int total_rows, const int* rows, const int* chunk_node, const int* chunk_start,
                                       const int* chunk_cnt, const int* chunk_slot, const int* wave_off, int n_waves, const void* src,
                                       int64_t ld_src, int width, void* dst, int64_t ld_dst, float* heavy, void* stream) {
    if (n_chunks <= 0 || n_waves <= 0) return 0;
    if (width <= 0 || width % 256 || width > 1536 || ld_src % 8 || ld_dst % 8 || (uintptr_t)src % 16 || (uintptr_t)dst % 16) return -24;
    if (!rows || !chunk_node || !chunk_start || !chunk_cnt || !wave_off || !src || !dst || (chunk_slot && !heavy) || total_rows <= 0) return -23;
    SegStreamArgs a;
    a.n_chunks = n_chunks; a.total_rows = total_rows; a.n_waves = n_waves;
    a.rows = rows; a.chunk_node = chunk_node; a.chunk_start = chunk_start; a.chunk_cnt = chunk_cnt; a.chunk_slot = chunk_slot;
    a.wave_off = wave_off; a.src = (const bf16_t*)src; a.ld_src = ld_src; a.dst = (bf16_t*)dst; a.ld_dst = ld_dst; a.heavy = heavy;
    hipStream_t s = static_cast<hipStream_t>(stream);
    const dim3 grid((unsigned)((n_waves + 3) / 4)), block(256);
#define GTOS_SEGS(S, H) hipLaunchKernelGGL((seg_sum_stream_kernel<S, H>), grid, block, 0, s, a.n_chunks, a.total_rows, a.n_waves, a.rows, \
        a.chunk_node, a.chunk_start, a.chunk_cnt, a.chunk_slot, a.wave_off, a.src, a.ld_src, a.dst, a.ld_dst, a.heavy)
    switch (width / 256) {
        case 1: GTOS_SEGS(0, true); break;
        case 2: GTOS_SEGS(1, false); break;
        case 3: GTOS_SEGS(1, true); break;
        case 4: GTOS_SEGS(2, false); break;
        case 5: GTOS_SEGS(2, true); break;
        default: GTOS_SEGS(3, false); break;
    }
#undef GTOS_SEGS
    GTOS_CHECK_LAUNCH();
    return 0;
}

extern "C" int gtos_segment_sum_finish(int n_heavy, const int* heavy_node, const float* heavy, int width, void* dst, int64_t ld_dst,
                                       void* stream) {
    if (n_heavy <= 0) return 0;
    if (width <= 0 || width % 8 || ld_dst % 8 || !heavy_node || !heavy || !dst) return -24;
    const int64_t n = (int64_t)n_heavy * (width / 8);
    hipLaunchKernelGGL(seg_finish_kernel, dim3((unsigned)((n + 255) / 256)), dim3(256), 0, static_cast<hipStream_t>(stream), n_heavy,
                       heavy_node, heavy, width, (bf16_t*)dst, ld_dst);
    GTOS_CHECK_LAUNCH();
    return 0;
}

extern "C" int gtos_segment_sum_ranges(int n_seg, const int* ranges, const void* src, int64_t ld_src, int width, void* dst, int64_t ld_dst,
                                       void* stream) {
    if (n_seg <= 0) return 0;
    if (width <= 0 || width % 8 || width > 1536 || ld_src % 8 || ld_dst % 8 || (uintptr_t)src % 16 || (uintptr_t)dst % 16) return -24;
    if (!ranges || !src || !dst) return -23;
    hipStream_t s = static_cast<hipStream_t>(stream);
    const dim3 grid((unsigned)((n_seg + 3) / 4)), block(256);
#define GTOS_SEG(S) hipLaunchKernelGGL(seg_sum_range_kernel<S>, grid, block, 0, s, n_seg, ranges, (const bf16_t*)src, ld_src, width, \
                                       (bf16_t*)dst, ld_dst)
    if (width <= 512) GTOS_SEG(1); else if (width <= 1024) GTOS_SEG(2); else GTOS_SEG(3);
#undef GTOS_SEG
    GTOS_CHECK_LAUNCH();
    return 0;
}

extern "C" int gtos_sqnorm(int64_t n, const float* g, float* out, void* stream) {
    if (n <= 0) return 0;
    hipStream_t s = static_cast<hipStream_t>(stream);
    hipLaunchKernelGGL(sqnorm_kernel, dim3(grid_for(n, 256 * 8)), dim3(256), 0, s, n, g, out);
    GTOS_CHECK_LAUNCH();
    return 0;
}

extern "C" int gtos_adam_step(int64_t n, float* p, const float* g, float* m, float* v, float lr, float beta1, float beta2,
                              float eps, float weight_decay, float gscale, const float* sqnorm, float max_norm,
                              void* bf16_mirror, void* stream) {
    if (n <= 0) return 0;
    hipStream_t s = static_cast<hipStream_t>(stream);
    hipLaunchKernelGGL(adam_kernel, dim3(grid_for(n, 256 * 4)), dim3(256), 0, s, n, p, g, m, v, lr, beta1, beta2, eps, weight_decay,
                       gscale, sqnorm, max_norm, (bf16_t*)bf16_mirror, (const float*)nullptr);
    GTOS_CHECK_LAUNCH();
    return 0;
}

extern "C" int gtos_adam_step_ctl(int64_t n, float* p, const float* g, float* m, float* v, const float* ctl, float beta1, float beta2,
                                  float eps, float weight_decay, float gscale, const float* sqnorm, float max_norm,
                                  void* bf16_mirror, void* stream) {
    if (n <= 0) return 0;
    if (!ctl) return -23;
    hipStream_t s = static_cast<hipStream_t>(stream);
    hipLaunchKernelGGL(adam_kernel, dim3(grid_for(n, 256 * 4)), dim3(256), 0, s, n, p, g, m, v, 0.f, beta1, beta2, eps, weight_decay,
                       gscale, sqnorm, max_norm, (bf16_t*)bf16_mirror, ctl);
    GTOS_CHECK_LAUNCH();
    return 0;
}

extern "C" int gtos_step_control(int phase, const float* loss, double* state, float* flag, int warmup_steps, int embed_dim,
                                 float* ctl, void* stream) {
    if ((phase != 0 && phase != 1) || !loss || !state || !flag || !ctl || warmup_steps < 1 || embed_dim < 1) return -23;
    hipLaunchKernelGGL(step_control_kernel, dim3(1), dim3(64), 0, static_cast<hipStream_t>(stream), phase, loss, state, flag,
                       (double)warmup_steps, (double)embed_dim, ctl);
    GTOS_CHECK_LAUNCH();
    return 0;
}

extern "C" int gtos_cast_f32_to_bf16(int64_t n, const float* src, void* dst, void* stream) {
    if (n <= 0) return 0;
    hipStream_t s = static_cast<hipStream_t>(stream);
    hipLaunchKernelGGL(cast_bf16_kernel, dim3(grid_for(n, 256 * 4)), dim3(256), 0, s, n, src, (bf16_t*)dst);
    GTOS_CHECK_LAUNCH();
    return 0;
}

extern "C" int gtos_transpose_batch_bf16(int n_mat, const int64_t* desc, const int* tile_start, int total_tiles, const void* src,
                                         void* dst, void* stream) {
    if (n_mat <= 0 || total_tiles <= 0) return 0;
    if (!desc || !tile_start || !src || !dst) return -23;
    hipLaunchKernelGGL(transpose_batch_kernel, dim3((unsigned)total_tiles), dim3(256), 0, static_cast<hipStream_t>(stream), n_mat, desc,
                       tile_start, (const bf16_t*)src, (bf16_t*)dst);
    GTOS_CHECK_LAUNCH();
    return 0;
}

extern "C" int gtos_set_seed_epoch(const void* epoch) {
    int rc = gtosi_gemm_set_seed_epoch(epoch);
    if (!rc) rc = gtosi_rel_attn_set_seed_epoch(epoch);
    if (!rc) rc = gtosi_rowops_set_seed_epoch(epoch);
    if (!rc) rc = gtosi_gru_step_set_seed_epoch(epoch);
    if (!rc) rc = gtosi_tokenenc_set_seed_epoch(epoch);
    return rc;
}

extern "C" int gtos_abi_version(void) { return 25; }

GTOS_SEED_EPOCH_SETTER(rowops)
```

### gtos_amd/gru.py

```python
import contextlib
import os

import torch

from . import _lib
from ._lib import call, dt, ptr, stream
from .ops import (gemm, compute_weight, next_seed, weight_t, _grad_target, _splitk, side_stream as _side_stream, side_ok, defer_side_join, _Timed,
                  embed_bwd_workspace, _workspace, WORKSPACE_BYTES, note_memory)


def _cell_fwd(A, hs, xg, hg, h, y, y_off_elems, ldy, hprev, gates, p, seed, drop_base):
    yp = None if y is None else y.data_ptr() + y_off_elems * y.element_size()
    call("gtos_gru_cell_fwd", dt(xg), A, hs, ptr(xg), ptr(hg), ptr(h), yp, ldy, ptr(hprev), ptr(gates),
         float(p), seed, drop_base, stream())


N_BIAS_PARTIALS = 1024

FUSE = "x"
SIDE_STREAM = os.environ.get("GTOS_GRU_SIDE", "1") != "0"
SIDE_MIN_ROWS = 200000


def _step_fwd(A, hs, x, xg, h_in, wi, b_ih, wh, b_hh, h_out, n_out, h_fin, gates, y, y_off_elems, ldy, p, seed, drop_base,
              h_idx=None, gf=None, gf_idx=None, gb=None, gb_idx=None, fin_idx=None, tag=None):
    yp = None if y is None else y.data_ptr() + y_off_elems * y.element_size()
    need_bi = x is not None or gf is not None
    name = tag or "gru_step_fwd_%s" % ("x" if x is not None else ("tables" if gf is not None else "xg"))
    units = A if tag is None else A * 2 * (x.shape[1] + hs + 4 * hs + hs + (hs if y is not None else 0))
    with _Timed(name, detail=True, units=units):
        _step_fwd_call(A, hs, x, xg, h_in, wi, b_ih, wh, b_hh, h_out, n_out, h_fin, gates, yp, ldy, p, seed, drop_base,
                       h_idx, gf, gf_idx, gb, gb_idx, need_bi, fin_idx)


def _step_fwd_call(A, hs, x, xg, h_in, wi, b_ih, wh, b_hh, h_out, n_out, h_fin, gates, yp, ldy, p, seed, drop_base,
                   h_idx, gf, gf_idx, gb, gb_idx, need_bi, fin_idx=None):
    call("gtos_gru_step_fwd", A, hs, ptr(x), 0 if x is None else x.stride(0), 0 if x is None else x.shape[1],
         ptr(wi) if x is not None else None, ptr(b_ih) if need_bi else None, ptr(xg),
         ptr(gf), ptr(gf_idx), ptr(gb), ptr(gb_idx), ptr(h_in), ptr(h_idx), ptr(wh), ptr(b_hh),
         ptr(h_out), n_out, ptr(h_fin), hs if h_fin is None else h_fin.stride(0), ptr(fin_idx), ptr(gates), yp, ldy,
         float(p), seed, drop_base, stream())


def _step_bwd(A, hs, d4_prev, rows_prev, wh_t, gates, hprev, dy_ptr, ldy, dh, d4, p, seed, drop_base, bpart, hprev_idx=None, hp_out=None,
              sum_idx=None, dh_src=None, zero_row=-1):
    with _Timed("gru_step_bwd_%s" % ("trie" if hprev_idx is not None else "rows"), detail=True, units=A):
        call("gtos_gru_step_bwd", A, hs, ptr(d4_prev), rows_prev if d4_prev is not None else 0, ptr(wh_t), ptr(gates), ptr(hprev),
             ptr(hprev_idx), dy_ptr, ldy, ptr(dh), dt(dh), dh.stride(0), ptr(d4), float(p), seed, drop_base,
             ptr(bpart), N_BIAS_PARTIALS if bpart is not None else 0, ptr(hp_out), ptr(sum_idx), ptr(dh_src), int(zero_row), stream())


def _cell_bwd(A, hs, gates, hprev, dy, dy_off_elems, ldy, dh, dxg, dhg, p, seed, drop_base, bpart):
    dyp = None if dy is None else dy.data_ptr() + dy_off_elems * dy.element_size()
    call("gtos_gru_cell_bwd", dt(gates), A, hs, ptr(gates), ptr(hprev), dyp, ldy, ptr(dh), ptr(dxg), ptr(dhg),
         float(p), seed, drop_base, ptr(bpart), 0 if bpart is None else bpart.shape[0], stream())


class BiGRUFinalFn(torch.autograd.Function):

    @staticmethod
    def forward(ctx, x, batch_sizes, hs, num_layers, p_drop, *weights):
        L, R = len(batch_sizes), batch_sizes[0]
        offs = [0]
        for a in batch_sizes:
            offs.append(offs[-1] + a)
        N = offs[-1]
        assert x.shape[0] == N
        dev, dtp = x.device, x.dtype
        inp = x.contiguous()
        saved = []
        finals = None
        for l in range(num_layers):
            last = l == num_layers - 1
            Y = None if last else torch.empty((N, 2 * hs), dtype=dtp, device=dev)
            seed = next_seed() if (p_drop > 0 and not last) else 0
            pl = p_drop if not last else 0.0
            finals = []
            layer_saved = []
            for direction in (0, 1):
                w_ih, w_hh, b_ih, b_hh = weights[l * 8 + direction * 4: l * 8 + direction * 4 + 4]
                wi, wh = compute_weight(w_ih, dtp), compute_weight(w_hh, dtp)
                gates = torch.empty((N, 4 * hs), dtype=dtp, device=dev)
                hprev = torch.empty((N, hs), dtype=dtp, device=dev)
                steps = range(L) if direction == 0 else range(L - 1, -1, -1)
                fuse = FUSE if (dtp == torch.bfloat16 and hs % 64 == 0 and inp.shape[1] % 8 == 0) else "off"
                if fuse != "off":
                    h = torch.empty((R, hs), dtype=dtp, device=dev)
                    xg = None if fuse == "x" else gemm(inp, wi, trans_b=True, bias=b_ih.detach())
                    bi, bh = b_ih.detach(), b_hh.detach()
                    if direction == 0:
                        hprev[:R].zero_()
                    else:
                        for t in range(L):
                            lo = batch_sizes[t + 1] if t + 1 < L else 0
                            if batch_sizes[t] > lo:
                                hprev[offs[t] + lo: offs[t] + batch_sizes[t]].zero_()
                    for t in steps:
                        A, off = batch_sizes[t], offs[t]
                        nxt = t + 1 if direction == 0 else t - 1
                        if 0 <= nxt < L:
                            h_out, n_out = hprev[offs[nxt]:], min(A, batch_sizes[nxt])
                        else:
                            h_out, n_out = h, A
                        _step_fwd(A, hs, inp[off:off + A] if fuse == "x" else None, None if fuse == "x" else xg[off:off + A],
                                  hprev[off:off + A], wi, bi, wh, bh, h_out, n_out, h, gates[off:off + A],
                                  Y, off * 2 * hs + direction * hs, 2 * hs, pl, seed, off * 2 * hs + direction * hs)
                else:
                    xg = gemm(inp, wi, trans_b=True, bias=b_ih.detach())
                    h = torch.zeros((R, hs), dtype=dtp, device=dev)
                    hg = torch.empty((R, 3 * hs), dtype=dtp, device=dev)
                    for t in steps:
                        A, off = batch_sizes[t], offs[t]
                        gemm(h[:A], wh, trans_b=True, bias=b_hh.detach(), out=hg[:A])
                        _cell_fwd(A, hs, xg[off:off + A], hg, h, Y, off * 2 * hs + direction * hs, 2 * hs,
                                  hprev[off:off + A], gates[off:off + A], pl, seed, off * 2 * hs + direction * hs)
                finals.append(h)
                layer_saved.append((weight_t(w_ih, wi), weight_t(w_hh, wh), gates, hprev))
            saved.append((inp, seed, pl, layer_saved))
            inp = Y
        ctx.cfg = (batch_sizes, offs, hs, num_layers, weights, saved)
        return torch.cat(finals, 1)

    @staticmethod
    def backward(ctx, d_out):
        with _Timed("relation_gru_bwd"):
            return BiGRUFinalFn._backward(ctx, d_out)

    @staticmethod
    def _backward(ctx, d_out):
        batch_sizes, offs, hs, num_layers, weights, saved = ctx.cfg
        L, R, N = len(batch_sizes), batch_sizes[0], offs[-1]
        d_out = d_out.contiguous()
        dev = d_out.device
        grads = [None] * len(weights)
        used_side = False
        dY = None
        for l in range(num_layers - 1, -1, -1):
            inp, seed, pl, layer_saved = saved[l]
            dtp = inp.dtype
            d_inp = None
            for direction in (0, 1):
                wi_t, wh_t, gates, hprev = layer_saved[direction]
                base = l * 8 + direction * 4
                w_ih, w_hh, b_ih, b_hh = weights[base:base + 4]
                steps = range(L - 1, -1, -1) if direction == 0 else range(L)
                want_bias = b_ih.requires_grad or b_hh.requires_grad
                fused = FUSE != "off" and dtp == torch.bfloat16 and hs % 64 == 0
                dh_dt = dtp if fused else torch.float32
                if l == num_layers - 1:
                    dh = d_out[:, direction * hs:(direction + 1) * hs].to(dh_dt).contiguous()
                else:
                    dh = torch.zeros((R, hs), dtype=dh_dt, device=dev)
                if fused:
                    d4 = torch.empty((N, 4 * hs), dtype=dtp, device=dev)
                    bpart = torch.zeros((N_BIAS_PARTIALS, 4 * hs), dtype=torch.float32, device=dev) if want_bias else None
                    prev = None
                    for t in steps:
                        A, off = batch_sizes[t], offs[t]
                        dyp = None if dY is None else dY.data_ptr() + (off * 2 * hs + direction * hs) * dY.element_size()
                        _step_bwd(A, hs, None if prev is None else d4[offs[prev]:], 0 if prev is None else batch_sizes[prev], wh_t,
                                  gates[off:off + A], hprev[off:off + A], dyp, 2 * hs, dh, d4[off:off + A], pl, seed,
                                  off * 2 * hs + direction * hs, bpart)
                        prev = t
                    dxg = d4[:, :3 * hs]
                    w_jobs = ((w_hh, d4[:, :2 * hs], hprev, 1, slice(0, 2 * hs)), (w_hh, d4[:, 3 * hs:], hprev, 1, slice(2 * hs, 3 * hs)),
                              (w_ih, dxg, inp, 0, slice(0, 3 * hs)))
                else:
                    dxg = torch.empty((N, 3 * hs), dtype=dtp, device=dev)
                    dhg = torch.empty((N, 3 * hs), dtype=dtp, device=dev)
                    fuse_bias = (256 % (hs // 8) == 0) and want_bias
                    bpart = torch.zeros((N_BIAS_PARTIALS, 4 * hs), dtype=torch.float32, device=dev) if fuse_bias else None
                    for t in steps:
                        A, off = batch_sizes[t], offs[t]
                        _cell_bwd(A, hs, gates[off:off + A], hprev[off:off + A], dY, off * 2 * hs + direction * hs, 2 * hs,
                                  dh, dxg[off:off + A], dhg[off:off + A], pl, seed, off * 2 * hs + direction * hs, bpart)
                        gemm(dhg[off:off + A], wh_t, trans_b=True, out=dh[:A], accumulate=True)
                    w_jobs = ((w_hh, dhg, hprev, 1, slice(0, 3 * hs)), (w_ih, dxg, inp, 0, slice(0, 3 * hs)))
                for (wt, _, _, slot, _) in w_jobs:
                    if wt.requires_grad and _grad_target(wt) is None and grads[base + slot] is None:
                        grads[base + slot] = torch.zeros(wt.shape, dtype=torch.float32, device=dev)
                for (bt, slot) in ((b_hh, 3), (b_ih, 2)):
                    if bt.requires_grad and _grad_target(bt) is None:
                        grads[base + slot] = torch.zeros(bt.shape, dtype=torch.float32, device=dev)
                main = torch.cuda.current_stream(dev)
                side = _side_stream(dev) if (SIDE_STREAM and side_ok(dev) and fused and N >= SIDE_MIN_ROWS) else main
                if side is not main:
                    side.wait_stream(main)
                    for t_ in (d4, bpart, hprev, inp):
                        if t_ is not None:
                            t_.record_stream(side)
                with torch.cuda.stream(side):
                    for (wt, dyv, xin, slot, rows) in w_jobs:
                        if wt.requires_grad:
                            tgt = _grad_target(wt)
                            if tgt is None:
                                tgt = grads[base + slot]
                            nrow = rows.stop - rows.start
                            gemm(dyv, xin, trans_a=True, out=tgt[rows], accumulate=True, splitk=_splitk(nrow, wt.shape[1], N))
                    bsum = bpart.sum(0) if bpart is not None else None
                    for (bt, slot) in ((b_hh, 3), (b_ih, 2)):
                        if bt.requires_grad:
                            tgt = _grad_target(bt)
                            if tgt is None:
                                tgt = grads[base + slot]
                            if bsum is not None:
                                tgt[:2 * hs] += bsum[:2 * hs]
                                tgt[2 * hs:] += bsum[2 * hs:3 * hs] if slot == 2 else bsum[3 * hs:]
                            else:
                                dyv = dhg if slot == 3 else dxg
                                call("gtos_colsum", dt(dyv), N, 3 * hs, 3 * hs, ptr(dyv), ptr(tgt), stream())
                used_side = used_side or side is not main
                if l > 0 or ctx.needs_input_grad[0]:
                    if d_inp is None:
                        d_inp = gemm(dxg, wi_t, trans_b=True)
                    else:
                        gemm(dxg, wi_t, trans_b=True, out=d_inp, accumulate=True)
            dY = d_inp
        if used_side:
            if all(gr is None for gr in grads):
                defer_side_join(dev)
            else:
                torch.cuda.current_stream(dev).wait_stream(_side_stream(dev))
        return (dY if ctx.needs_input_grad[0] else None, None, None, None, None) + tuple(grads)


class PackPlan(object):

    def __init__(self, batch_sizes, order32, order64=None):
        self.batch_sizes = [int(a) for a in batch_sizes if a > 0]
        self.offs = [0]
        for a in self.batch_sizes:
            self.offs.append(self.offs[-1] + a)
        self.L, self.N = len(self.batch_sizes), self.offs[-1]
        self.order32 = order32
        self.order64 = order64 if order64 is not None else order32.to(torch.int64)
        self.offs_dev = torch.tensor(self.offs, dtype=torch.int32).to(order32.device, non_blocking=True)

    @staticmethod
    def of_trie(trie):
        plan = getattr(trie, "_pack_plan", None)
        if plan is None or plan.order32.device != trie.seq_order32.device:
            plan = trie._pack_plan = PackPlan(trie.batch_sizes, trie.seq_order32, trie.seq_order)
        return plan

    @staticmethod
    def of_lengths(lengths, max_len):
        sorted_len, order = torch.sort(lengths, descending=True, stable=True)
        bs = (sorted_len.unsqueeze(0) > torch.arange(max_len, device=lengths.device).unsqueeze(1)).sum(1).tolist()
        return PackPlan(bs, order.to(torch.int32), order)


def _step_bwd_fused(A, hs, d4_prev, rows_prev, wh_t, gates, hprev, dy_ptr, ldy, dh, d4, p, seed, drop_base, bpart,
                    wi_t=None, dinp=None, n_in=0, dinp_acc=False, p_in=0.0, seed_in=0, in_drop_base=0, tag="gru_step_bwd_packed"):
    rp = rows_prev if d4_prev is not None else 0
    both = min(A, rp) if dinp is not None else 0
    nbytes = 2 * (A * (4 * hs + hs + 2 * hs + 4 * hs + (hs if dy_ptr else 0)) + both * 4 * hs
                  + ((rp - both) * 3 * hs if dinp is not None else min(A, rp) * 3 * hs) + (rp * n_in * (2 if dinp_acc else 1) if dinp is not None else 0))
    with _Timed(tag, detail=True, units=nbytes):
        call("gtos_gru_step_bwd_fused", A, hs, ptr(d4_prev), rows_prev if d4_prev is not None else 0, ptr(wh_t), ptr(gates), ptr(hprev), None,
             dy_ptr, ldy, ptr(dh), 0 if dh is None else dt(dh), hs if dh is None else dh.stride(0), ptr(d4), float(p), seed, drop_base,
             ptr(bpart), N_BIAS_PARTIALS if bpart is not None else 0, None, None, None, -1,
             ptr(wi_t), ptr(dinp), 0 if dinp is None else dinp.stride(0), n_in, int(dinp_acc), float(p_in), seed_in, in_drop_base, stream())


D4_INPLACE = os.environ.get("GTOS_GRU_D4_INPLACE", "auto")
D4_INPLACE_MIN_BYTES = 8 << 30


class PackedPathGRUFn(torch.autograd.Function):

    @staticmethod
    def forward(ctx, bank, plan, table, dim_pad, p_embed, hs, p_layer, *weights):
        dev, dtp = table.device, torch.bfloat16
        bs, offs, L, N = plan.batch_sizes, plan.offs, plan.L, plan.N
        R = bank.shape[1]
        if L == 0 or R == 0:
            ctx.cfg = False
            return torch.zeros((R, 2 * hs), dtype=dtp, device=dev)
        V, dim = table.shape
        tab = table.detach()
        want_table = table.requires_grad and ctx.needs_input_grad[2]
        Vp = (V + 7) // 8 * 8
        X = torch.empty((N, dim_pad), dtype=dtp, device=dev)
        onehot = torch.empty((N, Vp), dtype=dtp, device=dev) if (want_table and V <= 256) else None
        tokens = torch.empty((N,), dtype=torch.int64, device=dev) if (want_table and V > 256) else None
        seed_e = next_seed() if p_embed > 0 else 0
        call("gtos_embed_packed_paths", dt(X), L, R, N, ptr(bank), ptr(plan.order32), ptr(plan.offs_dev), ptr(tab), dim, dim_pad, ptr(X),
             float(p_embed), seed_e, ptr(onehot), Vp, ptr(tokens), stream())
        fin = (torch.empty if bs[0] == R else torch.zeros)((R, 2 * hs), dtype=dtp, device=dev)
        park = [torch.empty((bs[0], hs), dtype=dtp, device=dev) for _ in (0, 1)]
        inp, saved = X, []
        for l in range(2):
            last = l == 1
            Y = None if last else torch.empty((N, 2 * hs), dtype=dtp, device=dev)
            seed = next_seed() if (p_layer > 0 and not last) else 0
            pl = p_layer if not last else 0.0
            layer_saved = []
            bufs = [(torch.empty((N, 4 * hs), dtype=dtp, device=dev), torch.empty((N, hs), dtype=dtp, device=dev)) for _ in (0, 1)]
            wts = []
            for direction in (0, 1):
                w_ih, w_hh, b_ih, b_hh = weights[l * 8 + direction * 4: l * 8 + direction * 4 + 4]
                wi, wh = compute_weight(w_ih, dtp), compute_weight(w_hh, dtp)
                if wi.shape[1] != inp.shape[1]:
                    wi = torch.nn.functional.pad(wi.detach(), (0, inp.shape[1] - wi.shape[1]))
                    wi_t = wi.t().contiguous()
                else:
                    wi_t = weight_t(w_ih, wi)
                wts.append((wi, wh, wi_t, weight_t(w_hh, wh), b_ih.detach(), b_hh.detach()))
            for direction in (0, 1):
                wi, wh, wi_t, wh_t, bi, bh = wts[direction]
                gates, hprev = bufs[direction]
                if direction == 0:
                    hprev[:bs[0]].zero_()
                else:
                    for t in range(L):
                        lo = bs[t + 1] if t + 1 < L else 0
                        if bs[t] > lo:
                            hprev[offs[t] + lo: offs[t] + bs[t]].zero_()
                h_fin = fin[:, direction * hs:(direction + 1) * hs] if last else park[direction]
                for t in (range(L) if direction == 0 else range(L - 1, -1, -1)):
                    A, off = bs[t], offs[t]
                    nxt = t + 1 if direction == 0 else t - 1
                    if 0 <= nxt < L:
                        h_out, n_out = hprev[offs[nxt]:], min(A, bs[nxt])
                    else:
                        h_out, n_out = None, 0
                    _step_fwd(A, hs, inp[off:off + A], None, hprev[off:off + A], wi, bi, wh, bh, h_out, n_out, h_fin, gates[off:off + A],
                              Y, off * 2 * hs + direction * hs, 2 * hs, pl, seed, off * 2 * hs + direction * hs,
                              fin_idx=plan.order32 if last else None, tag="gru_step_fwd_packed_l%d" % l)
                layer_saved.append((wi_t, wh_t, gates, hprev))
            saved.append((inp, seed, pl, layer_saved))
            inp = Y
        ctx.cfg = (plan, table, dim_pad, p_embed, seed_e, hs, weights, saved, onehot, tokens)
        return fin

    @staticmethod
    def backward(ctx, d_out):
        with _Timed("relation_gru_bwd"):
            return PackedPathGRUFn._backward(ctx, d_out)

    @staticmethod
    def _backward(ctx, d_out):
        if ctx.cfg is False:
            return (None,) * len(ctx.needs_input_grad)
        if ctx.cfg is None:
            raise RuntimeError("PackedPathGRUFn: backward called a second time -- the saved gates and states are released piece by piece "
                               "during the first (retain_graph is not supported on this path)")
        plan, table, dim_pad, p_embed, seed_e, hs, weights, saved, onehot, tokens = ctx.cfg
        bs, offs, L, N = plan.batch_sizes, plan.offs, plan.L, plan.N
        dev, dtp = d_out.device, torch.bfloat16
        dfin = d_out.to(dtp).index_select(0, plan.order64)
        grads = [None] * len(weights)
        for base in (8, 12, 0, 4):
            for slot in range(4):
                wt_ = weights[base + slot]
                if wt_.requires_grad and _grad_target(wt_) is None:
                    grads[base + slot] = torch.zeros(wt_.shape, dtype=torch.float32, device=dev)
        want_table = onehot is not None or tokens is not None
        main = torch.cuda.current_stream(dev)
        used_side, held = False, None
        dY = None
        dX = None
        saved = [list(e) for e in saved]
        ctx.cfg = None
        for l in (1, 0):
            inp, seed, pl, layer_saved = saved[l]
            saved[l] = None
            layer_saved = list(layer_saved)
            n_in = inp.shape[1]
            want_dinp = l == 1 or want_table
            d_in = torch.empty((N, n_in), dtype=dtp, device=dev) if want_dinp else None
            for direction in (0, 1):
                wi_t, wh_t, gates, hprev = layer_saved[direction]
                layer_saved[direction] = None
                base = l * 8 + direction * 4
                w_ih, w_hh, b_ih, b_hh = weights[base:base + 4]
                want_bias = b_ih.requires_grad or b_hh.requires_grad
                dh = dfin[:, direction * hs:(direction + 1) * hs] if l == 1 else torch.zeros((bs[0], hs), dtype=dtp, device=dev)
                in_place = D4_INPLACE == "1" or (D4_INPLACE != "0" and gates.numel() * gates.element_size() >= D4_INPLACE_MIN_BYTES)
                d4 = gates if in_place else torch.empty((N, 4 * hs), dtype=dtp, device=dev)
                note_memory(dev)
                bpart = torch.zeros((N_BIAS_PARTIALS, 4 * hs), dtype=torch.float32, device=dev) if want_bias else None
                rb = dict(wi_t=wi_t, n_in=n_in, dinp_acc=direction == 1, p_in=p_embed if l == 0 else 0.0,
                          seed_in=seed_e if l == 0 else 0) if want_dinp else None
                tag = "gru_step_bwd_packed_l%d" % l
                prev = None
                for t in (range(L - 1, -1, -1) if direction == 0 else range(L)):
                    A, off = bs[t], offs[t]
                    dyp = None if dY is None else dY.data_ptr() + (off * 2 * hs + direction * hs) * dY.element_size()
                    kw = {} if (rb is None or prev is None) else dict(rb, dinp=d_in[offs[prev]:], in_drop_base=offs[prev] * n_in)
                    _step_bwd_fused(A, hs, None if prev is None else d4[offs[prev]:], 0 if prev is None else bs[prev], wh_t,
                                    gates[off:off + A], hprev[off:off + A], dyp, 2 * hs, dh, d4[off:off + A], pl, seed,
                                    off * 2 * hs + direction * hs, bpart, tag=tag, **kw)
                    prev = t
                if rb is not None:
                    _step_bwd_fused(0, hs, d4[offs[prev]:], bs[prev], wh_t, None, None, None, 2 * hs, None, None, 0.0, 0, 0, None, tag=tag,
                                    **dict(rb, dinp=d_in[offs[prev]:], in_drop_base=offs[prev] * n_in))
                del gates
                side = _side_stream(dev) if (SIDE_STREAM and side_ok(dev) and N >= SIDE_MIN_ROWS) else main
                if held is not None:
                    main.wait_stream(_side_stream(dev))
                    held = None
                if side is not main:
                    side.wait_stream(main)
                    held = (d4, bpart, hprev, inp)
                with torch.cuda.stream(side):
                    tg_ih = _grad_target(w_ih) if w_ih.requires_grad else None
                    tg_hh = _grad_target(w_hh) if w_hh.requires_grad else None
                    tg_ih = grads[base] if (tg_ih is None and w_ih.requires_grad) else tg_ih
                    tg_hh = grads[base + 1] if (tg_hh is None and w_hh.requires_grad) else tg_hh
                    scr_ih = torch.zeros(w_ih.shape, dtype=torch.float32, device=dev) if tg_ih is None else tg_ih
                    scr_hh = torch.zeros(w_hh.shape, dtype=torch.float32, device=dev) if tg_hh is None else tg_hh
                    if (tg_ih is not None or tg_hh is not None) and w_ih.shape[1] % 4 == 0:
                        with _Timed("gru_dw_grouped_l%d" % l, detail=True, units=2 * N * 3 * hs * (w_ih.shape[1] + hs)):
                            ws = _workspace(dev)
                            call("gtos_gru_weight_grads", N, hs, n_in, w_ih.shape[1], ptr(d4), ptr(inp), inp.stride(0), ptr(hprev), hprev.stride(0),
                                 ptr(scr_ih), scr_ih.stride(0), ptr(scr_hh), scr_hh.stride(0), ptr(ws), ws.numel() * 4, stream())
                    elif tg_ih is not None or tg_hh is not None:
                        for (tg, dyv, xin, rows) in ((tg_hh, d4[:, :2 * hs], hprev, slice(0, 2 * hs)), (tg_hh, d4[:, 3 * hs:], hprev, slice(2 * hs, 3 * hs)),
                                                     (tg_ih, d4[:, :3 * hs], inp, slice(0, 3 * hs))):
                            if tg is None:
                                continue
                            sk = _splitk(rows.stop - rows.start, xin.shape[1], N)
                            if tg.shape[1] == xin.shape[1]:
                                gemm(dyv, xin, trans_a=True, out=tg[rows], accumulate=True, splitk=sk)
                            else:
                                tg[rows] += gemm(dyv, xin, trans_a=True, out_dtype=torch.float32, splitk=sk)[:, :tg.shape[1]]
                    if want_bias:
                        _acc_bias_grads(grads, base, b_ih, b_hh, bpart.sum(0), hs)
                used_side = used_side or side is not main
                del d4, hprev, bpart
            del inp
            if l == 1:
                dY = d_in
            else:
                dX, dY = d_in, None
        dtab = None
        if want_table:
            tgt = _grad_target(table)
            if tgt is None:
                tgt = dtab = torch.zeros(table.shape, dtype=torch.float32, device=dev)
            V, dim = table.shape
            if onehot is not None:
                part = gemm(onehot, dX, trans_a=True, out_dtype=torch.float32, splitk=_splitk(onehot.shape[1], dim_pad, N))
                tgt += part[:V, :dim]
            else:
                ws = embed_bwd_workspace(N, V, dim_pad, dev)
                call("gtos_embed_rows_bwd", dt(dX), N, V, dim, dim_pad, ptr(tokens), ptr(dX), ptr(tgt), 0.0, 0, ptr(ws),
                     0 if ws is None else ws.numel() * 4, stream())
        if used_side:
            if dtab is None and all(gr is None for gr in grads):
                defer_side_join(dev, list(t_ for t_ in (held or ()) if t_ is not None))
            else:
                main.wait_stream(_side_stream(dev))
        return (None, None, dtab, None, None, None, None) + tuple(grads)


def packed_path_gru(bank, plan, table, dim_pad, p_embed, hs, p_layer, weights):
    return PackedPathGRUFn.apply(bank, plan, table, dim_pad, float(p_embed), hs, float(p_layer), *weights)


def bigru_final(x_packed, batch_sizes, hs, num_layers, p_drop, weights):
    return BiGRUFinalFn.apply(x_packed, tuple(batch_sizes), hs, num_layers, float(p_drop), *weights)


TRIE = os.environ.get("GTOS_GRU_TRIE", "1") != "0"
TRIE_SIDE = False
TRIE_L0_OVERLAP = True
EMBED_GRAD_GEMM = True
TRIE_SUM_INDEX = True


SEG_STREAM = True


def _seg_rows(side, src, width, dst, src2=None, dst2=None):
    heavy = torch.zeros((2 if src2 is not None else 1, max(1, side.n_heavy), width), dtype=torch.float32, device=src.device)
    if SEG_STREAM and src2 is None and width % 256 == 0:
        with _Timed("segment_sum_rows", detail=True, units=int(side.rows.numel())):
            call("gtos_segment_sum_stream", side.n_chunks, int(side.rows.numel()), ptr(side.rows), ptr(side.chunk_node), ptr(side.chunk_start),
                 ptr(side.chunk_cnt), ptr(side.chunk_slot), ptr(side.wave_off), side.n_waves, ptr(src), src.stride(0), width, ptr(dst),
                 dst.stride(0), ptr(heavy[0]), stream())
            call("gtos_segment_sum_finish", side.n_heavy, ptr(side.heavy_node), ptr(heavy[0]), width, ptr(dst), dst.stride(0), stream())
        return
    with _Timed("segment_sum_rows", detail=True, units=int(side.rows.numel()) * (2 if src2 is not None else 1)):
        call("gtos_segment_sum_rows", side.n_chunks, ptr(side.rows), ptr(side.chunk_node), ptr(side.chunk_start), ptr(side.chunk_cnt),
             ptr(side.chunk_slot), ptr(src), ptr(src2), src.stride(0), width, ptr(dst), ptr(dst2), dst.stride(0),
             ptr(heavy[0]), ptr(heavy[1]) if src2 is not None else None, stream())
        call("gtos_segment_sum_finish", side.n_heavy, ptr(side.heavy_node), ptr(heavy[0]), width, ptr(dst), dst.stride(0), stream())
        if src2 is not None:
            call("gtos_segment_sum_finish", side.n_heavy, ptr(side.heavy_node), ptr(heavy[1]), width, ptr(dst2), dst2.stride(0), stream())


def _seg_ranges(n_seg, ranges, src, width, dst):
    call("gtos_segment_sum_ranges", n_seg, ptr(ranges), ptr(src), src.stride(0), width, ptr(dst), dst.stride(0), stream())


def _acc_weight_grad(grads, slot, wt, dy, x, rows=None, cols=None):
    if not wt.requires_grad:
        return
    tgt = _grad_target(wt)
    if tgt is None:
        if grads[slot] is None:
            grads[slot] = torch.zeros(wt.shape, dtype=torch.float32, device=dy.device)
        tgt = grads[slot]
    if rows is not None:
        tgt = tgt[rows]
    if cols is not None:
        tgt = tgt[:, cols]
    gemm(dy, x, trans_a=True, out=tgt, accumulate=True, splitk=_splitk(dy.shape[1], x.shape[1], dy.shape[0]))


def _acc_bias_grads(grads, base, b_ih, b_hh, bsum, hs):
    for bt, slot in ((b_hh, 3), (b_ih, 2)):
        if not bt.requires_grad:
            continue
        tgt = _grad_target(bt)
        if tgt is None:
            if grads[base + slot] is None:
                grads[base + slot] = torch.zeros(bt.shape, dtype=torch.float32, device=bsum.device)
            tgt = grads[base + slot]
        tgt[:2 * hs] += bsum[:2 * hs]
        tgt[2 * hs:] += bsum[2 * hs:3 * hs] if slot == 2 else bsum[3 * hs:]


class TrieBiGRUFn(torch.autograd.Function):

    @staticmethod
    def forward(ctx, trie, table, dim_pad, p_embed, hs, p_layer, *weights):
        dev, dtp = table.device, torch.bfloat16
        L, R, N = trie.L, trie.R, trie.N
        bs = trie.batch_sizes
        offs = [0]
        for a in bs:
            offs.append(offs[-1] + a)
        sides = (trie.pf, trie.sf)
        dim = table.shape[1]
        tab = table.detach()
        l0 = []
        main = torch.cuda.current_stream(dev)
        aux = _side_stream(dev) if (TRIE_L0_OVERLAP and table.is_cuda and side_ok(dev) and N >= SIDE_MIN_ROWS) else main
        seeds = [(next_seed() if p_embed > 0 else 0, next_seed() if p_layer > 0 else 0) for _ in sides]
        if aux is not main:
            aux.wait_stream(main)
        for d, side in enumerate(sides):
            with torch.cuda.stream(aux if d == 1 else main):
                n = side.n_nodes
                w_ih, w_hh, b_ih, b_hh = weights[d * 4: d * 4 + 4]
                wi, wh = compute_weight(w_ih, dtp), compute_weight(w_hh, dtp)
                seed_e, seed_y = seeds[d]
                X = torch.empty((n, dim_pad), dtype=dtp, device=dev)
                call("gtos_embed_rows_fwd", dt(X), n, dim, dim_pad, ptr(side.tok), ptr(tab), ptr(X), float(p_embed), seed_e, stream())
                H = torch.empty((n + 1, hs), dtype=dtp, device=dev)
                H[n].zero_()
                gates = torch.empty((n, 4 * hs), dtype=dtp, device=dev)
                Y = torch.empty((n, hs), dtype=dtp, device=dev) if p_layer > 0 else None
                bi, bh = b_ih.detach(), b_hh.detach()
                for k in range(L):
                    lo, hi = side.level_off[k], side.level_off[k + 1]
                    if hi > lo:
                        _step_fwd(hi - lo, hs, X[lo:hi], None, H, wi, bi, wh, bh, H[lo:hi], hi - lo, None, gates[lo:hi],
                                  Y, lo * hs, hs, p_layer, seed_y, lo * hs, h_idx=side.par[lo:hi])
                l0.append((X, H, gates, Y, seed_e, seed_y, weight_t(w_ih, wi), weight_t(w_hh, wh)))
        if aux is not main:
            main.wait_stream(aux)
        src = [l0[d][3] if p_layer > 0 else l0[d][1][:sides[d].n_nodes] for d in (0, 1)]
        fin = torch.empty((R, 2 * hs), dtype=dtp, device=dev)
        l1 = []
        tables = []
        for d in (0, 1):
            wi = compute_weight(weights[8 + d * 4], dtp)
            Gf = torch.empty((sides[0].n_nodes, 3 * hs), dtype=dtp, device=dev)
            Gb = torch.empty((sides[1].n_nodes, 3 * hs), dtype=dtp, device=dev)
            gemm(src[0], wi[:, :hs], trans_b=True, out=Gf)
            gemm(src[1], wi[:, hs:], trans_b=True, out=Gb)
            tables.append((Gf, Gb))
        for d in (0, 1):
            w_ih, w_hh, b_ih, b_hh = weights[8 + d * 4: 8 + d * 4 + 4]
            wi, wh = compute_weight(w_ih, dtp), compute_weight(w_hh, dtp)
            Gf, Gb = tables[d]
            gates = torch.empty((N, 4 * hs), dtype=dtp, device=dev)
            hprev = torch.empty((N, hs), dtype=dtp, device=dev)
            h = fin[:, d * hs:(d + 1) * hs]
            bi, bh = b_ih.detach(), b_hh.detach()
            if d == 0:
                hprev[:R].zero_()
            else:
                for t in range(L):
                    lo = bs[t + 1] if t + 1 < L else 0
                    if bs[t] > lo:
                        hprev[offs[t] + lo: offs[t] + bs[t]].zero_()
            for t in (range(L) if d == 0 else range(L - 1, -1, -1)):
                A, off = bs[t], offs[t]
                nxt = t + 1 if d == 0 else t - 1
                if 0 <= nxt < L:
                    h_out, n_out = hprev[offs[nxt]:], min(A, bs[nxt])
                else:
                    h_out, n_out = None, 0
                _step_fwd(A, hs, None, None, hprev[off:off + A], None, bi, wh, bh, h_out, n_out, h, gates[off:off + A],
                          None, 0, hs, 0.0, 0, 0, gf=Gf, gf_idx=trie.row_pf[off:off + A], gb=Gb, gb_idx=trie.row_sf[off:off + A],
                          fin_idx=trie.seq_order32)
            l1.append((gates, hprev, wi, weight_t(w_hh, wh)))
        ctx.cfg = (trie, table, dim_pad, p_embed, hs, p_layer, weights, l0, l1, offs)
        return fin

    @staticmethod
    def backward(ctx, d_out):
        with _Timed("relation_gru_bwd"):
            return TrieBiGRUFn._backward(ctx, d_out)

    @staticmethod
    def _backward(ctx, d_out):
        trie, table, dim_pad, p_embed, hs, p_layer, weights, l0, l1, offs = ctx.cfg
        dev, dtp = d_out.device, torch.bfloat16
        L, R, N = trie.L, trie.R, trie.N
        bs = trie.batch_sizes
        sides = (trie.pf, trie.sf)
        d_out = d_out.to(dtp).index_select(0, trie.seq_order)
        grads = [None] * len(weights)
        src = [l0[d][3] if p_layer > 0 else l0[d][1][:sides[d].n_nodes] for d in (0, 1)]
        dsrc = [None, None]
        main = torch.cuda.current_stream(dev)
        aux = _side_stream(dev) if (TRIE_SIDE and SIDE_STREAM and side_ok(dev) and N >= SIDE_MIN_ROWS) else main
        use_side = aux is not main

        keep = []

        def on_side(*tensors):
            if use_side:
                aux.wait_stream(main)
                keep.extend(t_ for t_ in tensors if t_ is not None)
            return torch.cuda.stream(aux)
        for base in (8, 12, 0, 4):
            for slot in range(4):
                wt_ = weights[base + slot]
                if wt_.requires_grad and _grad_target(wt_) is None and grads[base + slot] is None:
                    grads[base + slot] = torch.zeros(wt_.shape, dtype=torch.float32, device=dev)
        dGs = [[None, None], [None, None]]
        wis = [l1[0][2], l1[1][2]]
        for d in (0, 1):
            gates, hprev, wi, wh_t = l1[d]
            base = 8 + d * 4
            w_ih, w_hh, b_ih, b_hh = weights[base:base + 4]
            want_bias = b_ih.requires_grad or b_hh.requires_grad
            dh = d_out[:, d * hs:(d + 1) * hs]
            d4 = torch.empty((N, 4 * hs), dtype=dtp, device=dev)
            bpart = torch.zeros((N_BIAS_PARTIALS, 4 * hs), dtype=torch.float32, device=dev) if want_bias else None
            prev = None
            for t in (range(L - 1, -1, -1) if d == 0 else range(L)):
                A, off = bs[t], offs[t]
                _step_bwd(A, hs, None if prev is None else d4[offs[prev]:], 0 if prev is None else bs[prev], wh_t,
                          gates[off:off + A], hprev[off:off + A], None, hs, dh, d4[off:off + A], 0.0, 0, 0, bpart)
                prev = t
            with on_side(d4, hprev, bpart):
                _acc_weight_grad(grads, base + 1, w_hh, d4[:, :2 * hs], hprev, rows=slice(0, 2 * hs))
                _acc_weight_grad(grads, base + 1, w_hh, d4[:, 3 * hs:], hprev, rows=slice(2 * hs, 3 * hs))
                if want_bias:
                    _acc_bias_grads(grads, base, b_ih, b_hh, bpart.sum(0), hs)
            for s_, side_t in enumerate(sides):
                dGs[s_][d] = torch.empty((side_t.n_nodes, 3 * hs), dtype=dtp, device=dev)
                _seg_rows(side_t, d4, 3 * hs, dGs[s_][d])
            if not use_side:
                l1[d] = None
            del d4, gates, hprev, bpart
        for s_, side_t in enumerate(sides):
            dG = dGs[s_]
            cols = slice(0, hs) if s_ == 0 else slice(hs, 2 * hs)
            with on_side(dG[0], dG[1], src[s_]):
                for d in (0, 1):
                    w_ih, wi = weights[8 + d * 4], wis[d]
                    _acc_weight_grad(grads, 8 + d * 4, w_ih, dG[d], src[s_], cols=cols)
                    wt = weight_t(w_ih, wi[:, cols], rows=("cols", s_))
                    if dsrc[s_] is None:
                        dsrc[s_] = gemm(dG[d], wt, trans_b=True)
                    else:
                        gemm(dG[d], wt, trans_b=True, out=dsrc[s_], accumulate=True)
        if use_side:
            main.wait_stream(aux)
        del dGs
        keep.clear()
        dtab = None
        if table.requires_grad and _grad_target(table) is None:
            dtab = torch.zeros(table.shape, dtype=torch.float32, device=dev)
        l0_overlap = TRIE_L0_OVERLAP and side_ok(dev) and not use_side and N >= SIDE_MIN_ROWS
        emb_parts = []
        aux0 = _side_stream(dev) if l0_overlap else main
        if l0_overlap:
            aux0.wait_stream(main)
        for d, side in enumerate(sides):
          with torch.cuda.stream(aux0 if d == 1 else main):
            X, H, gates, Y, seed_e, seed_y, wi_t, wh_t = l0[d]
            n = side.n_nodes
            base = d * 4
            w_ih, w_hh, b_ih, b_hh = weights[base:base + 4]
            want_bias = b_ih.requires_grad or b_hh.requires_grad
            hp = torch.empty((n, hs), dtype=dtp, device=dev)
# ... 84 lines not shown
```

### include/gtos_hip.h

```cpp
#ifndef GTOS_HIP_H
#define GTOS_HIP_H
#include <stdint.h>

#ifdef __cplusplus
extern "C" {
#endif

#define GTOS_F32 0
#define GTOS_BF16 1

int gtos_abi_version(void);

int gtos_gemm(int in_dtype, int out_dtype, int transA, int transB, int M, int N, int K,
              const void* A, int64_t lda, const void* B, int64_t ldb, void* C, int64_t ldc,
              const float* bias, int relu, float p_drop, uint64_t seed, int accumulate, int splitk,
              void* workspace, int64_t workspace_bytes, void* stream);

int gtos_rel_attn_fwd(int dtype, int mode, int T, int S, int B, int H, int d,
                      const void* q, int64_t ldq, const void* k, int64_t ldk, const void* v, int64_t ldv,
                      const void* rel, const int* idx_q, const uint8_t* key_pad, const uint8_t* attn_mask,
                      float scale, float p_drop, uint64_t seed,
                      void* o, int64_t ldo, float* lse, float* w, void* stream);

int gtos_rel_attn_bwd(int dtype, int mode, int T, int S, int B, int H, int d,
                      const void* q, int64_t ldq, const void* k, int64_t ldk, const void* v, int64_t ldv,
                      const void* rel, const int* idx_q, const int* idx_k,
                      const uint8_t* key_pad, const uint8_t* attn_mask,
                      float scale, float p_drop, uint64_t seed,
                      const void* o, int64_t ldo, const float* lse, const float* w,
                      const void* d_o, int64_t lddo, const float* dw,
                      void* dq, int64_t lddq, void* dk, int64_t lddk, void* dv, int64_t lddv,
                      void* d_rel, int64_t ld_drel, float* pd, float* gs, void* stream);

int gtos_rel_attn_bwd_bank(int dtype, int n, int B, int H, int d,
                           const void* q, int64_t ldq, const void* k, int64_t ldk,
                           const void* bank, const float* gs,
                           const int* pair_sorted, const int* chunk_type, const int* chunk_start,
                           const int* chunk_count, const int* chunk_slot, const int* xcd_off, int nchunks,
                           void* d_bank, int64_t ld_dbank, float* heavy, void* stream);

int gtos_pathtrie_dev_workspace(int64_t R, int64_t N, int64_t* bytes_out);
int gtos_pathtrie_dev_phase_a(int L, int64_t R, const int64_t* bank, const int64_t* length, void** common, void** pf, void** sf,
                              int32_t* sizes, void* workspace, size_t workspace_bytes, void* stream);
int gtos_pathtrie_dev_phase_b(int64_t R, int64_t N, int n_pf, int n_sf, int chunk, int rows_per_wave, void** common, void** pf,
                              void** sf, int32_t* sizes, void* workspace, size_t workspace_bytes, void* stream);

int gtos_relbatch_dev_workspace(int64_t total, int64_t* bytes_out);
int gtos_relbatch_dev_phase_a(const int64_t* geom, void** tab, void* workspace, size_t workspace_bytes, void* stream);
int gtos_relbatch_dev_phase_b(const int64_t* geom, int64_t R, void** tab, void* workspace, size_t workspace_bytes, void* stream);
int gtos_relbatch_dev_all_count(const int64_t* geom, void** tab, void* workspace, size_t workspace_bytes, void* stream);
int gtos_relbatch_dev_all_keys(const int64_t* geom, void** tab, void* workspace, size_t workspace_bytes, void* stream);
int gtos_relbatch_dev_all_fill(const int64_t* geom, int64_t R, void** tab, void* workspace, size_t workspace_bytes, void* stream);

int gtos_relindex_dev_workspace(int64_t n, int64_t* bytes_out);
int gtos_relindex_dev_phase_a(const int64_t* geom, void** tab, void* workspace, size_t workspace_bytes, void* stream);
int gtos_relindex_dev_phase_b(const int64_t* geom, int64_t nchunks, void** tab, void* workspace, size_t workspace_bytes, void* stream);

int gtos_ln_residual_fwd(int dtype, int rows, int d, const void* x, const void* r, float p_drop, uint64_t seed,
                         const float* gamma, const float* beta, float eps, void* y, float* mean, float* rstd, void* stream);
int gtos_ln_residual_bwd(int dtype, int rows, int d, const void* dy, const void* x, const void* r, float p_drop,
                         uint64_t seed, const float* gamma, const float* mean, const float* rstd,
                         void* dx, void* dr, float* dgamma, float* dbeta, void* stream);

int gtos_ln_residual_fwd2(int x_dtype, int r_dtype, int y_dtype, int rows, int d, const void* x, const void* r, float p_drop,
                          uint64_t seed, const float* gamma, const float* beta, float eps, void* y, void* y2_bf16,
                          float* mean, float* rstd, void* stream);
int gtos_ln_residual_bwd2(int x_dtype, int r_dtype, int y_dtype, int rows, int d, const void* dy, const void* dy2_bf16,
                          const void* x, const void* r, float p_drop, uint64_t seed, const float* gamma, const float* mean,
                          const float* rstd, void* dx, void* dr, float* dgamma, float* dbeta, void* stream);

int gtos_relu_dropout_bwd(int dtype, int64_t n, void* dh, const void* h, float p_drop, void* stream);

int gtos_colsum(int dtype, int rows, int N, int64_t ld, const void* dy, float* out, void* stream);

int gtos_gru_cell_fwd(int dtype, int rows, int hs, const void* xg, const void* hg, void* h, void* y, int64_t ldy,
                      void* hprev_save, void* gates, float p_drop, uint64_t seed, int64_t drop_base, void* stream);
int gtos_gru_step_fwd(int rows, int hs, const void* x, int64_t ldx, int in_dim, const void* w_ih, const float* b_ih,
                      const void* xg, const void* gf, const int* gf_idx, const void* gb, const int* gb_idx,
                      const void* h_in, const int* h_idx, const void* w_hh, const float* b_hh,
                      void* h_out, int n_out, void* h_fin, int64_t ld_fin, const int* fin_idx, void* gates, void* y, int64_t ldy,
                      float p_drop, uint64_t seed, int64_t drop_base, void* stream);

int gtos_gru_step_bwd(int rows, int hs, const void* d4_prev, int rows_prev, const void* w_hh_t,
                      const void* gates, const void* hprev, const int* hprev_idx, const void* dy, int64_t ldy, void* dh, int dh_dtype,
                      int64_t ld_dh, void* d4, float p_drop, uint64_t seed, int64_t drop_base, float* bias_partials, int n_partials,
                      void* hprev_out, const int* sum_idx, const void* dh_src, int zero_row, void* stream);

int gtos_gru_step_bwd_fused(int rows, int hs, const void* d4_prev, int rows_prev, const void* w_hh_t,
                            const void* gates, const void* hprev, const int* hprev_idx, const void* dy, int64_t ldy, void* dh, int dh_dtype,
                            int64_t ld_dh, void* d4, float p_drop, uint64_t seed, int64_t drop_base, float* bias_partials, int n_partials,
                            void* hprev_out, const int* sum_idx, const void* dh_src, int zero_row,
                            const void* w_ih_t, void* dinp, int64_t ld_dinp, int n_in, int dinp_accumulate, float p_in, uint64_t seed_in,
                            int64_t in_drop_base, void* stream);

int gtos_gru_weight_grads(int rows, int hs, int in_dim, int in_valid, const void* d4, const void* x, int64_t ldx, const void* hprev, int64_t ldh,
                          float* dwih, int64_t ld_dwih, float* dwhh, int64_t ld_dwhh, void* workspace, int64_t workspace_bytes, void* stream);

int gtos_gemm_tn_batch(int n, const void* const* A, const int64_t* lda, const int* M, const void* const* B, const int64_t* ldb, const int* N,
                       const int* K, float* const* C, const int64_t* ldc, float* const* bias, void* stream);

int gtos_segment_sum_rows(int n_chunks, const int* rows, const int* chunk_node, const int* chunk_start, const int* chunk_cnt,
                          const int* chunk_slot, const void* src, const void* src2, int64_t ld_src, int width,
                          void* dst, void* dst2, int64_t ld_dst, float* heavy, float* heavy2, void* stream);
int gtos_segment_sum_stream(int n_chunks, int total_rows, const int* rows, const int* chunk_node, const int* chunk_start,
                            const int* chunk_cnt, const int* chunk_slot, const int* wave_off, int n_waves, const void* src,
                            int64_t ld_src, int width, void* dst, int64_t ld_dst, float* heavy, void* stream);
int gtos_segment_sum_finish(int n_heavy, const int* heavy_node, const float* heavy, int width, void* dst, int64_t ld_dst,
                            void* stream);
int gtos_segment_sum_ranges(int n_seg, const int* ranges, const void* src, int64_t ld_src, int width, void* dst, int64_t ld_dst,
                            void* stream);

int gtos_gru_cell_bwd(int dtype, int rows, int hs, const void* gates, const void* hprev, const void* dy, int64_t ldy,
                      float* dh, void* dxg, void* dhg, float p_drop, uint64_t seed, int64_t drop_base,
                      float* bias_partials, int n_partials, void* stream);

int gtos_relation_gather_mean(int dtype, int64_t P, int K, int d, const void* bank, const int64_t* idx, int zero_row0,
                              void* out, void* stream);

int gtos_embed_rows_fwd(int dtype, int64_t n, int dim, int dim_pad, const int64_t* tok, const float* table, void* out,
                        float p_drop, uint64_t seed, void* stream);
int gtos_embed_rows_bwd(int dtype, int64_t n, int V, int dim, int dim_pad, const int64_t* tok, const void* dout,
                        float* dtable, float p_drop, uint64_t seed, float* workspace, int64_t workspace_bytes, void* stream);

int gtos_embed_packed_paths(int dtype, int L, int R, int64_t n_rows, const int64_t* bank, const int* order, const int* offs,
                            const float* table, int dim, int dim_pad, void* x, float p_drop, uint64_t seed, void* onehot, int vp,
                            int64_t* tokens, void* stream);

int gtos_highway_fwd(int dtype, int64_t N, int D, const void* y, const void* x, void* out, void* stream);
int gtos_highway_bwd(int dtype, int64_t N, int D, const void* y, const void* x, const void* dout, void* dy, void* dx, void* stream);
int gtos_max_relu_fwd(int dtype, int64_t N, int L, int F, const void* y, void* out, uint8_t* arg, void* stream);
int gtos_max_relu_bwd(int dtype, int64_t N, int L, int F, const void* out, const uint8_t* arg, const void* dout, void* dy, void* stream);
int gtos_token_row_fwd(int dtype, int64_t N, int Cc, int Ct, int Cp, const void* feat, const int64_t* tok, const float* table,
                       void* out, float p_drop, uint64_t seed, void* stream);
int gtos_token_row_bwd(int dtype, int64_t N, int Cc, int Ct, int Cp, const void* dout, const int64_t* tok, void* dfeat,
                       float* dtable, float p_drop, uint64_t seed, void* stream);

int gtos_sqnorm(int64_t n, const float* g, float* out, void* stream);
int gtos_adam_step(int64_t n, float* p, const float* g, float* m, float* v, float lr, float beta1, float beta2,
                   float eps, float weight_decay, float gscale, const float* sqnorm, float max_norm,
                   void* bf16_mirror, void* stream);
int gtos_cast_f32_to_bf16(int64_t n, const float* src, void* dst, void* stream);
int gtos_transpose_batch_bf16(int n_mat, const int64_t* desc, const int* tile_start, int total_tiles, const void* src, void* dst,
                              void* stream);

int gtos_step_control(int phase, const float* loss, double* state, float* flag, int warmup_steps, int embed_dim,
                      float* ctl, void* stream);

int gtos_set_seed_epoch(const void* epoch);
int gtos_adam_step_ctl(int64_t n, float* p, const float* g, float* m, float* v, const float* ctl, float beta1, float beta2,
                       float eps, float weight_decay, float gscale, const float* sqnorm, float max_norm,
                       void* bf16_mirror, void* stream);

int gtos_copy_nll_fwd(int dtype, int T, int B, int V, int S, const void* logits, int64_t ld_logits, const void* div,
                      const float* align, const int64_t* cp_seq, const int64_t* target, int64_t pad_idx,
                      float* nll, float* lse, float* p_tgt, void* stream);
int gtos_copy_nll_bwd(int dtype, int T, int B, int V, int S, const void* logits, int64_t ld_logits, const void* div,
                      const float* align, const int64_t* cp_seq, const int64_t* target, int64_t pad_idx,
                      const float* lse, const float* p_tgt, const float* d_nll, void* d_logits, void* d_div,
                      float* d_align, void* stream);
int gtos_copy_ll_fwd(int dtype, int T, int B, int V, int S, int tot_ext, const void* logits, int64_t ld_logits,
                     const void* div, const float* align, const int64_t* cp_seq, float* ll, void* stream);

int gtos_copy_nll_ls_prep(int B, int S, int V, const int64_t* cp_seq, int* ws, int64_t ws_words, void* stream);
int gtos_copy_nll_ls_fwd(int dtype, int T, int B, int V, int S, const void* logits, int64_t ld_logits, const void* div,
                         const float* align, const int64_t* target, int64_t pad_idx, float eps, const int* ws, int64_t ws_words,
                         float* loss, float* lse, float* sums, void* stream);
int gtos_copy_nll_ls_bwd(int dtype, int T, int B, int V, int S, const void* logits, int64_t ld_logits, const void* div,
                         const float* align, const int64_t* target, int64_t pad_idx, float eps, const int* ws, int64_t ws_words,
                         const float* lse, const float* sums, const float* d_loss, void* d_logits, void* d_div, float* d_align,
                         void* stream);

int gtos_copy_eval_fwd(int dtype, int T, int B, int V, int S, const void* logits, int64_t ld_logits, const void* div,
                       const float* align, const int64_t* cp_seq, const int64_t* target, int64_t pad_idx, float* nll,
                       int* pred, float* p_pred, void* stream);
int gtos_eval_accumulate(int T, int B, const float* nll, const int* pred, const int64_t* target, int64_t pad_idx,
                         double* sent_nll, int* sent_tokens, int* sent_correct, double* totals, void* stream);

int gtos_beam_topk(int rows, int tot, int k, const float* ll, int64_t ld, float* val, int* idx, void* stream);
int gtos_beam_advance(int B, int k, int t, int V, int tot, int min_time_step, int max_time_step, const float* topv,
                      const int* topi, const uint8_t* flag_shared, const uint8_t* flag_local, double* slot_score,
                      int* beam_state, int* bp_parent, int* bp_token, int* comp_step, int* comp_parent,
                      double* comp_score, int* active, void* stream);
int gtos_beam_reorder(int n_caches, void* const* src, void* const* dst, int64_t row_bytes, int N, int k, int t,
                      int max_time_step, const int* bp_parent, const int* bp_token, const int* beam_state,
                      const int* active, int V, int tot, const int64_t* tok_shared, const int64_t* tok_local,
                      const int64_t* char_shared, const int64_t* char_local, int C, int64_t dead_tok,
                      const int64_t* dead_char, int64_t* tok_out, int64_t* char_out, void* stream);

int gtos_sample_step(int N, int k, int t, int V, int tot, int min_time_step, int max_time_step, float temperature, int top_k,
                     float top_p, uint64_t seed, const float* ll, int64_t ld, const uint8_t* flag_shared,
                     const uint8_t* flag_local, const uint8_t* owned_local, double* score, int* slot_state, int* tokens,
                     int* active, const int64_t* tok_shared, const int64_t* tok_local, const int64_t* char_shared,
                     const int64_t* char_local, int C, int64_t dead_tok, const int64_t* dead_char, int64_t* tok_out,
                     int64_t* char_out, void* stream);

#ifdef __cplusplus
}
#endif
#endif
```

Measured before the change: 846.0.

## Skip recurrent GEMM for zero-hidden rows in packed GRU steps

Result: no change. 848.8, median of 5 (+0.3%).

```diff
diff --git a/gtos_amd/_lib.py b/gtos_amd/_lib.py
--- a/gtos_amd/_lib.py
+++ b/gtos_amd/_lib.py
@@ -6,7 +6,7 @@
 
 _HERE = os.path.dirname(os.path.abspath(__file__))
 LIB_PATH = os.path.join(_HERE, "csrc", "libgtos_hip.so")
-ABI_VERSION = 25
+ABI_VERSION = 26
 
 c_p, c_i, c_l, c_f, c_u64 = ctypes.c_void_p, ctypes.c_int, ctypes.c_int64, ctypes.c_float, ctypes.c_uint64
 
@@ -37,10 +37,10 @@
     "gtos_colsum": [c_i, c_i, c_i, c_l, c_p, c_p, c_p],
     "gtos_gru_cell_fwd": [c_i, c_i, c_i, c_p, c_p, c_p, c_p, c_l, c_p, c_p, c_f, c_u64, c_l, c_p],
     "gtos_gru_step_fwd": [c_i, c_i, c_p, c_l, c_i, c_p, c_p, c_p, c_p, c_p, c_p, c_p, c_p, c_p, c_p, c_p, c_p, c_i, c_p, c_l, c_p, c_p, c_p, c_l,
-                          c_f, c_u64, c_l, c_p],
+                          c_f, c_u64, c_l, c_p, c_i],
     "gtos_gru_step_bwd": [c_i, c_i, c_p, c_i, c_p, c_p, c_p, c_p, c_p, c_l, c_p, c_i, c_l, c_p, c_f, c_u64, c_l, c_p, c_i, c_p, c_p, c_p, c_i, c_p],
     "gtos_gru_step_bwd_fused": [c_i, c_i, c_p, c_i, c_p, c_p, c_p, c_p, c_p, c_l, c_p, c_i, c_l, c_p, c_f, c_u64, c_l, c_p, c_i, c_p, c_p, c_p, c_i,
-                                c_p, c_p, c_l, c_i, c_i, c_f, c_u64, c_l, c_p],
+                                c_p, c_p, c_l, c_i, c_i, c_f, c_u64, c_l, c_p, c_i],
     "gtos_gru_weight_grads": [c_i, c_i, c_i, c_i, c_p, c_p, c_l, c_p, c_l, c_p, c_l, c_p, c_l, c_p, c_l, c_p],
     "gtos_gemm_tn_batch": [c_i, c_p, c_p, c_p, c_p, c_p, c_p, c_p, c_p, c_p, c_p, c_p],
     "gtos_embed_packed_paths": [c_i, c_i, c_i, c_l, c_p, c_p, c_p, c_p, c_i, c_i, c_p, c_f, c_u64, c_p, c_i, c_p, c_p],
@@ -80,6 +80,11 @@
     "gtos_adam_step_ctl": [c_l, c_p, c_p, c_p, c_p, c_p, c_f, c_f, c_f, c_f, c_f, c_p, c_f, c_p, c_p],
 }
 
+TRAILING_DEFAULTS = {
+    "gtos_gru_step_fwd": (-1,),
+    "gtos_gru_step_bwd_fused": (-1,),
+}
+
 _lib = None
 _load_lock = threading.Lock()
 
@@ -110,6 +115,11 @@
 
 
 def call(name, *args):
+    tail = TRAILING_DEFAULTS.get(name)
+    if tail is not None:
+        missing = len(SIGNATURES[name]) - len(args)
+        if 0 < missing <= len(tail):
+            args = args + tail[len(tail) - missing:]
     rc = getattr(load(), name)(*args)
     if rc != 0:
         raise GtosHipError("%s failed with code %d (%s)" % (
diff --git a/gtos_amd/csrc/gru_step.hip b/gtos_amd/csrc/gru_step.hip
--- a/gtos_amd/csrc/gru_step.hip
+++ b/gtos_amd/csrc/gru_step.hip
@@ -29,6 +29,7 @@
     int64_t ld_fin; const int* fin_idx;
     float p_drop; uint64_t seed; int64_t drop_base;
     int rows, hs; const void* zeros;
+    int zero_from;
 };
 
 __device__ __forceinline__ void dma_rows(const bf16_t* __restrict__ base, const U128* __restrict__ zeros, int64_t ld, int rows_total,
@@ -65,14 +66,14 @@
 
 struct RowSrc { const char* p[TM / 32]; int c[TM / 32]; };
 __device__ __forceinline__ RowSrc row_src(const bf16_t* __restrict__ base, int64_t ld, int rows_total, int row0, int wave, int lane,
-                                          const int* __restrict__ gather = nullptr, int zero_row = -1) {
+                                          const int* __restrict__ gather = nullptr, int zero_row = -1, int zero_from = 0x7fffffff) {
     RowSrc s;
 #pragma unroll
     for (int it = 0; it < TM / 32; ++it) {
         const int rl = (it * 4 + wave) * 8 + (lane >> 3);
         const int r = row0 + rl;
         s.c[it] = (lane & 7) ^ swz(rl);
-        const bool ok = r < rows_total;
+        const bool ok = r < rows_total && r < zero_from;
         const int64_t sr = (gather && ok) ? gather[r] : r;
         s.p[it] = (ok && sr != zero_row) ? reinterpret_cast<const char*>(base + sr * ld + s.c[it] * 8) : nullptr;
     }
@@ -214,7 +215,7 @@
             const bf16_t* xp = a.xg + (int64_t)m * 3 * hs + cb;
             ld16(xp, xr); ld16(xp + hs, xz); ld16(xp + 2 * hs, xn);
         }
-        ld16(a.h_in + (int64_t)(a.h_idx ? a.h_idx[m] : m) * hs + cb, hp);
+        ld16(m < a.zero_from ? a.h_in + (int64_t)(a.h_idx ? a.h_idx[m] : m) * hs + cb : static_cast<const bf16_t*>(a.zeros), hp);
         float gr[16], gz[16], gn[16], hn[16], o[16];
 #pragma unroll
         for (int i = 0; i < 16; ++i) {
@@ -228,9 +229,8 @@
         bf16_t* gp = a.gates + (int64_t)m * 4 * hs + cb;
         st16(gp, gr); st16(gp + hs, gz); st16(gp + 2 * hs, gn);
         st16(gp + 3 * hs, hn);
-        bf16_t* hdst = m < a.n_out ? a.h_out + (int64_t)m * hs + cb
-                                   : a.h_fin + (int64_t)(a.fin_idx ? a.fin_idx[m] : m) * a.ld_fin + cb;
-        st16(hdst, o);
+        if (m < a.n_out) st16(a.h_out + (int64_t)m * hs + cb, o);
+        else if (a.h_fin) st16(a.h_fin + (int64_t)(a.fin_idx ? a.fin_idx[m] : m) * a.ld_fin + cb, o);
         if (a.y) {
             if (a.p_drop > 0.f) {
 #pragma unroll
@@ -276,8 +276,8 @@
             __syncthreads();
         }
     }
-    {
-        const RowSrc hsrc = row_src(a.h_in, a.hs, a.rows, m0, wave, lane, a.h_idx);
+    if (m0 < a.zero_from) {
+        const RowSrc hsrc = row_src(a.h_in, a.hs, a.rows, m0, wave, lane, a.h_idx, -1, a.zero_from);
         const WSrc ws = w_src(a.hs, a.hs, c0, wave, lane);
         for (int k0 = 0; k0 < a.hs; k0 += BK) {
             dma_rows_at(hsrc, Z, k0, a.hs, As, wave);
@@ -306,7 +306,9 @@
     const int xcd = blockIdx.x & 7, sq = blockIdx.x >> 3;
     const int m0 = ((sq / nC) * 8 + xcd) * TMW, c0 = (sq % nC) * TC;
     if (m0 >= a.rows) return;
-    const int nkx = a.in_dim / BK, nk = nkx + hs / BK;
+    const bool zpanel = m0 >= a.zero_from, strad = !zpanel && a.zero_from < min(m0 + TMW, a.rows);
+    const int nkx = a.in_dim / BK, nkf = nkx + hs / BK;
+    const char* Zc = static_cast<const char*>(a.zeros);
     uint32_t axo[4], aho[4], bxo[3], bho[3];
 #pragma unroll
     for (int i = 0; i < 4; ++i) {
@@ -314,7 +316,7 @@
         const int r = min(m0 + rl, a.rows - 1) - m0;
         const uint32_t c = (uint32_t)(((lane & 7) ^ swz(rl)) << 4);
         axo[i] = (uint32_t)r * (uint32_t)(a.ldx * 2) + c;
-        aho[i] = (uint32_t)r * (uint32_t)(hs * 2) + c;
+        aho[i] = m0 + r >= a.zero_from ? ~0u : (uint32_t)r * (uint32_t)(hs * 2) + c;
     }
 #pragma unroll
     for (int i = 0; i < 3; ++i) {
@@ -339,15 +341,22 @@
 #define GTOS_DMA1(src, dst)                                                                                                   \
     __builtin_amdgcn_global_load_lds((const __attribute__((address_space(1))) void*)(src),                                    \
                                      (__attribute__((address_space(3))) void*)(dst), 16, 0, 0)
-#define GTOS_A2W3_DMA_A(slot, s_)                                                                                             \
+#define GTOS_A2W3_DMA_A(slot, s_, ZA_)                                                                                        \
     {                                                                                                                         \
         const int st_ = min((s_), nk - 1);                                                                                    \
         const bool px_ = st_ < nkx;                                                                                           \
         const char* ab_ = px_ ? Xb + st_ * ROWB : Hb + (st_ - nkx) * ROWB;                                                    \
-        GTOS_DMA1(ab_ + (px_ ? axo[0] : aho[0]), (slot) + (0 * 8 + wave) * 1024);                                             \
-        GTOS_DMA1(ab_ + (px_ ? axo[1] : aho[1]), (slot) + (1 * 8 + wave) * 1024);                                             \
-        GTOS_DMA1(ab_ + (px_ ? axo[2] : aho[2]), (slot) + (2 * 8 + wave) * 1024);                                             \
-        GTOS_DMA1(ab_ + (px_ ? axo[3] : aho[3]), (slot) + (3 * 8 + wave) * 1024);                                             \
+        if (ZA_ && strad && !px_) {                                                                                                \
+            GTOS_DMA1(aho[0] == ~0u ? Zc : ab_ + aho[0], (slot) + (0 * 8 + wave) * 1024);                                     \
+            GTOS_DMA1(aho[1] == ~0u ? Zc : ab_ + aho[1], (slot) + (1 * 8 + wave) * 1024);                                     \
+            GTOS_DMA1(aho[2] == ~0u ? Zc : ab_ + aho[2], (slot) + (2 * 8 + wave) * 1024);                                     \
+            GTOS_DMA1(aho[3] == ~0u ? Zc : ab_ + aho[3], (slot) + (3 * 8 + wave) * 1024);                                     \
+        } else {                                                                                                              \
+            GTOS_DMA1(ab_ + (px_ ? axo[0] : aho[0]), (slot) + (0 * 8 + wave) * 1024);                                         \
+            GTOS_DMA1(ab_ + (px_ ? axo[1] : aho[1]), (slot) + (1 * 8 + wave) * 1024);                                         \
+            GTOS_DMA1(ab_ + (px_ ? axo[2] : aho[2]), (slot) + (2 * 8 + wave) * 1024);                                         \
+            GTOS_DMA1(ab_ + (px_ ? axo[3] : aho[3]), (slot) + (3 * 8 + wave) * 1024);                                         \
+        }                                                                                                                     \
     }
 #define GTOS_A2W3_DMA_W(slot, s_)                                                                                             \
     {                                                                                                                         \
@@ -358,12 +367,12 @@
         GTOS_DMA1(bb_ + (px_ ? bxo[1] : bho[1]), (slot) + (1 * 8 + wave) * 1024);                                             \
         GTOS_DMA1(bb_ + (px_ ? bxo[2] : bho[2]), (slot) + (2 * 8 + wave) * 1024);                                             \
     }
-#define GTOS_A2W3_STEP(sa_, sw_, sa_n, sw_n, s_)                                                                              \
+#define GTOS_A2W3_STEP(sa_, sw_, sa_n, sw_n, s_, ZA_)                                                                         \
     {                                                                                                                         \
         GTOS_VMCNT_LDS(4);                                  \
         __builtin_amdgcn_s_barrier();                       \
         GTOS_A2W3_DMA_W(sw_n, (s_) + 1);                                                                                      \
-        GTOS_A2W3_DMA_A(sa_n, (s_) + 2);                                                                                      \
+        GTOS_A2W3_DMA_A(sa_n, (s_) + 2, ZA_);                                                                                 \
         {                                                                                                                     \
             _Pragma("unroll") for (int ks = 0; ks < 2; ++ks) {                                                                \
                 bf16x8_t fa[2], fb[12];                                                                                       \
@@ -388,18 +397,48 @@
         }                                                                                                                     \
     }
 
-    if (nk > 0) {
-        GTOS_A2W3_DMA_A(sa0, 0);
+    if (!zpanel && !strad) {
+        const int nk = nkf;
+        if (nk > 0) {
+            GTOS_A2W3_DMA_A(sa0, 0, 0);
+            GTOS_A2W3_DMA_W(sw0, 0);
+            GTOS_A2W3_DMA_A(sa1, 1, 0);
+        }
+        for (int s = 0; s + 6 <= nk; s += 6) {
+            GTOS_A2W3_STEP(sa0, sw0, sa2, sw1, s, 0);
+            GTOS_A2W3_STEP(sa1, sw1, sa0, sw0, s + 1, 0);
+            GTOS_A2W3_STEP(sa2, sw0, sa1, sw1, s + 2, 0);
+            GTOS_A2W3_STEP(sa0, sw1, sa2, sw0, s + 3, 0);
+            GTOS_A2W3_STEP(sa1, sw0, sa0, sw1, s + 4, 0);
+            GTOS_A2W3_STEP(sa2, sw1, sa1, sw0, s + 5, 0);
+        }
+    } else {
+        const int nk = zpanel ? nkx : nkf;
+        GTOS_A2W3_DMA_A(sa0, 0, 1);
         GTOS_A2W3_DMA_W(sw0, 0);
-        GTOS_A2W3_DMA_A(sa1, 1);
-    }
-    for (int s = 0; s + 6 <= nk; s += 6) {
-        GTOS_A2W3_STEP(sa0, sw0, sa2, sw1, s);
-        GTOS_A2W3_STEP(sa1, sw1, sa0, sw0, s + 1);
-        GTOS_A2W3_STEP(sa2, sw0, sa1, sw1, s + 2);
-        GTOS_A2W3_STEP(sa0, sw1, sa2, sw0, s + 3);
-        GTOS_A2W3_STEP(sa1, sw0, sa0, sw1, s + 4);
-        GTOS_A2W3_STEP(sa2, sw1, sa1, sw0, s + 5);
+        GTOS_A2W3_DMA_A(sa1, 1, 1);
+        int s = 0;
+        for (; s + 6 <= nk; s += 6) {
+            GTOS_A2W3_STEP(sa0, sw0, sa2, sw1, s, 1);
+            GTOS_A2W3_STEP(sa1, sw1, sa0, sw0, s + 1, 1);
+            GTOS_A2W3_STEP(sa2, sw0, sa1, sw1, s + 2, 1);
+            GTOS_A2W3_STEP(sa0, sw1, sa2, sw0, s + 3, 1);
+            GTOS_A2W3_STEP(sa1, sw0, sa0, sw1, s + 4, 1);
+            GTOS_A2W3_STEP(sa2, sw1, sa1, sw0, s + 5, 1);
+        }
+        if (s < nk) {
+            GTOS_A2W3_STEP(sa0, sw0, sa2, sw1, s, 1);
+            if (s + 1 < nk) {
+                GTOS_A2W3_STEP(sa1, sw1, sa0, sw0, s + 1, 1);
+                if (s + 2 < nk) {
+                    GTOS_A2W3_STEP(sa2, sw0, sa1, sw1, s + 2, 1);
+                    if (s + 3 < nk) {
+                        GTOS_A2W3_STEP(sa0, sw1, sa2, sw0, s + 3, 1);
+                        if (s + 4 < nk) GTOS_A2W3_STEP(sa1, sw0, sa0, sw1, s + 4, 1);
+                    }
+                }
+            }
+        }
     }
     GTOS_VMCNT(0);
 #undef GTOS_A2W3_STEP
@@ -568,6 +607,7 @@
     int rows, hs; const void* zeros;
     const bf16_t* wi_t; bf16_t* dinp; int64_t ld_dinp; int n_in; int dinp_acc;
     float p_in; uint64_t seed_in; int64_t in_drop_base;
+    int zero_from;
 };
 
 #define GTOS_DPP(v, ctrl) __builtin_bit_cast(float, __builtin_amdgcn_update_dpp(0, __builtin_bit_cast(int, (v)), (ctrl), 0xF, 0xF, true))
@@ -755,7 +795,7 @@
         const bf16_t* gp = a.gates + (int64_t)m * 4 * hs + cb;
         ld16(gp, gr); ld16(gp + hs, gz); ld16(gp + 2 * hs, gn);
         ld16(gp + 3 * hs, hn);
-        ld16(a.hprev + (int64_t)(a.hprev_idx ? a.hprev_idx[m] : m) * hs + cb, hp);
+        ld16(m < a.zero_from ? a.hprev + (int64_t)(a.hprev_idx ? a.hprev_idx[m] : m) * hs + cb : static_cast<const bf16_t*>(a.zeros), hp);
         float* dhp = static_cast<float*>(a.dh) + (int64_t)m * a.ld_dh + cb;
         bf16_t* dhb = static_cast<bf16_t*>(a.dh) + (int64_t)m * a.ld_dh + cb;
         if (a.sum_idx) {
@@ -829,13 +869,14 @@
                                  const void* xg, const void* gf, const int* gf_idx, const void* gb, const int* gb_idx,
                                  const void* h_in, const int* h_idx, const void* w_hh, const float* b_hh,
                                  void* h_out, int n_out, void* h_fin, int64_t ld_fin, const int* fin_idx, void* gates, void* y, int64_t ldy,
-                                 float p_drop, uint64_t seed, int64_t drop_base, void* stream) {
+                                 float p_drop, uint64_t seed, int64_t drop_base, void* stream, int zero_from) {
     if (rows <= 0) return 0;
     if (hs <= 0 || hs % TC) return -22;
+    if (zero_from < 0 || zero_from > rows) zero_from = rows;
+    const int mode = x ? 1 : (gf ? 2 : 0);
     if (!h_in || !w_hh || !b_hh || !gates) return -23;
-    if ((n_out > 0 && !h_out) || (n_out < rows && !h_fin)) return -23;
+    if ((n_out > 0 && !h_out) || (n_out < rows && !h_fin && mode == 2)) return -23;
     if (h_fin && (ld_fin < hs || ld_fin % 8)) return -25;
-    const int mode = x ? 1 : (gf ? 2 : 0);
     if (mode == 1) {
         if (!w_ih || !b_ih || in_dim <= 0 || in_dim % 8 || ldx % 8 || (uintptr_t)x % 16 || (uintptr_t)w_ih % 16) return -24;
     } else if (mode == 2) {
@@ -850,14 +891,14 @@
     a.h_in = (const bf16_t*)h_in; a.h_idx = h_idx; a.w_hh = (const bf16_t*)w_hh; a.b_hh = b_hh;
     a.h_out = (bf16_t*)h_out; a.n_out = n_out; a.h_fin = (bf16_t*)h_fin; a.gates = (bf16_t*)gates; a.y = (bf16_t*)y; a.ldy = ldy;
     a.ld_fin = ld_fin; a.fin_idx = fin_idx;
-    a.p_drop = p_drop; a.seed = seed; a.drop_base = drop_base; a.rows = rows; a.hs = hs;
+    a.p_drop = p_drop; a.seed = seed; a.drop_base = drop_base; a.rows = rows; a.hs = hs; a.zero_from = zero_from;
     a.zeros = gtos_zero_block();
     if (!a.zeros) return -5;
     const long long nM = (rows + TM - 1) / TM, nC = hs / TC;
     const long long nblk = ((nM + 7) / 8) * 8 * nC;
     if (nblk > 0x7fffffffLL) return -6;
     hipStream_t s = static_cast<hipStream_t>(stream);
-    if (mode == 2 && hs == 256 && !h_idx && !y && rows >= 16384) {
+    if (mode == 2 && hs == 256 && !h_idx && !y && rows >= 16384 && zero_from == rows) {
         constexpr int KT = 4;
         const size_t lds_bytes = (size_t)KT * B_BYTES + 4 * KT * P_ROWS * ROWB;
         static bool configured = false;
@@ -890,11 +931,12 @@
                                        float* bias_partials, int n_partials, void* hprev_out, const int* sum_idx, const void* dh_src,
                                        int zero_row,
                                        const void* w_ih_t, void* dinp, int64_t ld_dinp, int n_in, int dinp_accumulate, float p_in,
-                                       uint64_t seed_in, int64_t in_drop_base, void* stream) {
+                                       uint64_t seed_in, int64_t in_drop_base, void* stream, int zero_from) {
     const bool role_b = dinp != nullptr && d4_prev != nullptr && rows_prev > 0;
     if (rows <= 0 && !role_b) return 0;
     if (hs <= 0 || hs % TC) return -22;
     if (rows > 0) {
+        if (zero_from < 0 || zero_from > rows) zero_from = rows;
         if (!gates || !hprev || !dh || !d4 || (d4_prev && !w_hh_t)) return -23;
         if (sum_idx && (!dh_src || (uintptr_t)dh_src % 16)) return -23;
     }
@@ -911,7 +953,7 @@
     a.hp_out = (bf16_t*)hprev_out; a.sum_idx = sum_idx; a.dh_src = dh_src; a.zero_row = sum_idx ? zero_row : -1;
     a.wi_t = (const bf16_t*)w_ih_t; a.dinp = role_b ? (bf16_t*)dinp : nullptr; a.ld_dinp = ld_dinp; a.n_in = n_in; a.dinp_acc = dinp_accumulate;
     a.p_in = p_in; a.seed_in = seed_in; a.in_drop_base = in_drop_base;
-    a.p_drop = p_drop; a.seed = seed; a.drop_base = drop_base; a.rows = rows > 0 ? rows : 0; a.hs = hs;
+    a.p_drop = p_drop; a.seed = seed; a.drop_base = drop_base; a.rows = rows > 0 ? rows : 0; a.hs = hs; a.zero_from = rows > 0 ? zero_from : 0;
     a.zeros = gtos_zero_block();
     if (!a.zeros) return -5;
     const long long cover = role_b && rows_prev > a.rows ? rows_prev : a.rows;
@@ -929,7 +971,7 @@
                                  int n_partials, void* hprev_out, const int* sum_idx, const void* dh_src, int zero_row, void* stream) {
     return gtos_gru_step_bwd_fused(rows, hs, d4_prev, rows_prev, w_hh_t, gates, hprev, hprev_idx, dy, ldy, dh, dh_dtype, ld_dh, d4,
                                    p_drop, seed, drop_base, bias_partials, n_partials, hprev_out, sum_idx, dh_src, zero_row,
-                                   nullptr, nullptr, 0, 0, 0, 0.f, 0, 0, stream);
+                                   nullptr, nullptr, 0, 0, 0, 0.f, 0, 0, stream, -1);
 }
 
 GTOS_SEED_EPOCH_SETTER(gru_step)
diff --git a/gtos_amd/csrc/rowops.hip b/gtos_amd/csrc/rowops.hip
--- a/gtos_amd/csrc/rowops.hip
+++ b/gtos_amd/csrc/rowops.hip
@@ -1142,6 +1142,6 @@
     return rc;
 }
 
-extern "C" int gtos_abi_version(void) { return 25; }
+extern "C" int gtos_abi_version(void) { return 26; }
 
 GTOS_SEED_EPOCH_SETTER(rowops)
diff --git a/gtos_amd/gru.py b/gtos_amd/gru.py
--- a/gtos_amd/gru.py
+++ b/gtos_amd/gru.py
@@ -23,23 +23,23 @@
 
 
 def _step_fwd(A, hs, x, xg, h_in, wi, b_ih, wh, b_hh, h_out, n_out, h_fin, gates, y, y_off_elems, ldy, p, seed, drop_base,
-              h_idx=None, gf=None, gf_idx=None, gb=None, gb_idx=None, fin_idx=None, tag=None):
+              h_idx=None, gf=None, gf_idx=None, gb=None, gb_idx=None, fin_idx=None, tag=None, zero_from=-1):
     yp = None if y is None else y.data_ptr() + y_off_elems * y.element_size()
     need_bi = x is not None or gf is not None
     name = tag or "gru_step_fwd_%s" % ("x" if x is not None else ("tables" if gf is not None else "xg"))
     units = A if tag is None else A * 2 * (x.shape[1] + hs + 4 * hs + hs + (hs if y is not None else 0))
     with _Timed(name, detail=True, units=units):
         _step_fwd_call(A, hs, x, xg, h_in, wi, b_ih, wh, b_hh, h_out, n_out, h_fin, gates, yp, ldy, p, seed, drop_base,
-                       h_idx, gf, gf_idx, gb, gb_idx, need_bi, fin_idx)
+                       h_idx, gf, gf_idx, gb, gb_idx, need_bi, fin_idx, zero_from)
 
 
 def _step_fwd_call(A, hs, x, xg, h_in, wi, b_ih, wh, b_hh, h_out, n_out, h_fin, gates, yp, ldy, p, seed, drop_base,
-                   h_idx, gf, gf_idx, gb, gb_idx, need_bi, fin_idx=None):
+                   h_idx, gf, gf_idx, gb, gb_idx, need_bi, fin_idx=None, zero_from=-1):
     call("gtos_gru_step_fwd", A, hs, ptr(x), 0 if x is None else x.stride(0), 0 if x is None else x.shape[1],
          ptr(wi) if x is not None else None, ptr(b_ih) if need_bi else None, ptr(xg),
          ptr(gf), ptr(gf_idx), ptr(gb), ptr(gb_idx), ptr(h_in), ptr(h_idx), ptr(wh), ptr(b_hh),
          ptr(h_out), n_out, ptr(h_fin), hs if h_fin is None else h_fin.stride(0), ptr(fin_idx), ptr(gates), yp, ldy,
-         float(p), seed, drop_base, stream())
+         float(p), seed, drop_base, stream(), zero_from)
 
 
 def _step_bwd(A, hs, d4_prev, rows_prev, wh_t, gates, hprev, dy_ptr, ldy, dh, d4, p, seed, drop_base, bpart, hprev_idx=None, hp_out=None,
@@ -236,6 +236,11 @@
         self.order64 = order64 if order64 is not None else order32.to(torch.int64)
         self.offs_dev = torch.tensor(self.offs, dtype=torch.int32).to(order32.device, non_blocking=True)
 
+    def zero_from(self, direction, t):
+        if direction == 0:
+            return 0 if t == 0 else self.batch_sizes[t]
+        return self.batch_sizes[t + 1] if t + 1 < self.L else 0
+
     @staticmethod
     def of_trie(trie):
         plan = getattr(trie, "_pack_plan", None)
@@ -251,7 +256,7 @@
 
 
 def _step_bwd_fused(A, hs, d4_prev, rows_prev, wh_t, gates, hprev, dy_ptr, ldy, dh, d4, p, seed, drop_base, bpart,
-                    wi_t=None, dinp=None, n_in=0, dinp_acc=False, p_in=0.0, seed_in=0, in_drop_base=0, tag="gru_step_bwd_packed"):
+                    wi_t=None, dinp=None, n_in=0, dinp_acc=False, p_in=0.0, seed_in=0, in_drop_base=0, tag="gru_step_bwd_packed", zero_from=-1):
     rp = rows_prev if d4_prev is not None else 0
     both = min(A, rp) if dinp is not None else 0
     nbytes = 2 * (A * (4 * hs + hs + 2 * hs + 4 * hs + (hs if dy_ptr else 0)) + both * 4 * hs
@@ -260,7 +265,8 @@
         call("gtos_gru_step_bwd_fused", A, hs, ptr(d4_prev), rows_prev if d4_prev is not None else 0, ptr(wh_t), ptr(gates), ptr(hprev), None,
              dy_ptr, ldy, ptr(dh), 0 if dh is None else dt(dh), hs if dh is None else dh.stride(0), ptr(d4), float(p), seed, drop_base,
              ptr(bpart), N_BIAS_PARTIALS if bpart is not None else 0, None, None, None, -1,
-             ptr(wi_t), ptr(dinp), 0 if dinp is None else dinp.stride(0), n_in, int(dinp_acc), float(p_in), seed_in, in_drop_base, stream())
+             ptr(wi_t), ptr(dinp), 0 if dinp is None else dinp.stride(0), n_in, int(dinp_acc), float(p_in), seed_in, in_drop_base, stream(),
+             zero_from)
 
 
 D4_INPLACE = os.environ.get("GTOS_GRU_D4_INPLACE", "auto")
@@ -288,7 +294,6 @@
         call("gtos_embed_packed_paths", dt(X), L, R, N, ptr(bank), ptr(plan.order32), ptr(plan.offs_dev), ptr(tab), dim, dim_pad, ptr(X),
              float(p_embed), seed_e, ptr(onehot), Vp, ptr(tokens), stream())
         fin = (torch.empty if bs[0] == R else torch.zeros)((R, 2 * hs), dtype=dtp, device=dev)
-        park = [torch.empty((bs[0], hs), dtype=dtp, device=dev) for _ in (0, 1)]
         inp, saved = X, []
         for l in range(2):
             last = l == 1
@@ -314,10 +319,10 @@
                     hprev[:bs[0]].zero_()
                 else:
                     for t in range(L):
-                        lo = bs[t + 1] if t + 1 < L else 0
+                        lo = plan.zero_from(1, t)
                         if bs[t] > lo:
                             hprev[offs[t] + lo: offs[t] + bs[t]].zero_()
-                h_fin = fin[:, direction * hs:(direction + 1) * hs] if last else park[direction]
+                h_fin = fin[:, direction * hs:(direction + 1) * hs] if last else None
                 for t in (range(L) if direction == 0 else range(L - 1, -1, -1)):
                     A, off = bs[t], offs[t]
                     nxt = t + 1 if direction == 0 else t - 1
@@ -327,7 +332,7 @@
                         h_out, n_out = None, 0
                     _step_fwd(A, hs, inp[off:off + A], None, hprev[off:off + A], wi, bi, wh, bh, h_out, n_out, h_fin, gates[off:off + A],
                               Y, off * 2 * hs + direction * hs, 2 * hs, pl, seed, off * 2 * hs + direction * hs,
-                              fin_idx=plan.order32 if last else None, tag="gru_step_fwd_packed_l%d" % l)
+                              fin_idx=plan.order32 if last else None, tag="gru_step_fwd_packed_l%d" % l, zero_from=plan.zero_from(direction, t))
                 layer_saved.append((wi_t, wh_t, gates, hprev))
             saved.append((inp, seed, pl, layer_saved))
             inp = Y
@@ -391,7 +396,7 @@
                     kw = {} if (rb is None or prev is None) else dict(rb, dinp=d_in[offs[prev]:], in_drop_base=offs[prev] * n_in)
                     _step_bwd_fused(A, hs, None if prev is None else d4[offs[prev]:], 0 if prev is None else bs[prev], wh_t,
                                     gates[off:off + A], hprev[off:off + A], dyp, 2 * hs, dh, d4[off:off + A], pl, seed,
-                                    off * 2 * hs + direction * hs, bpart, tag=tag, **kw)
+                                    off * 2 * hs + direction * hs, bpart, tag=tag, zero_from=plan.zero_from(direction, t), **kw)
                     prev = t
                 if rb is not None:
                     _step_bwd_fused(0, hs, d4[offs[prev]:], bs[prev], wh_t, None, None, None, 2 * hs, None, None, 0.0, 0, 0, None, tag=tag,
diff --git a/include/gtos_hip.h b/include/gtos_hip.h
--- a/include/gtos_hip.h
+++ b/include/gtos_hip.h
@@ -79,7 +79,7 @@
                       const void* xg, const void* gf, const int* gf_idx, const void* gb, const int* gb_idx,
                       const void* h_in, const int* h_idx, const void* w_hh, const float* b_hh,
                       void* h_out, int n_out, void* h_fin, int64_t ld_fin, const int* fin_idx, void* gates, void* y, int64_t ldy,
-                      float p_drop, uint64_t seed, int64_t drop_base, void* stream);
+                      float p_drop, uint64_t seed, int64_t drop_base, void* stream, int zero_from);
 
 int gtos_gru_step_bwd(int rows, int hs, const void* d4_prev, int rows_prev, const void* w_hh_t,
                       const void* gates, const void* hprev, const int* hprev_idx, const void* dy, int64_t ldy, void* dh, int dh_dtype,
@@ -91,7 +91,7 @@
                             int64_t ld_dh, void* d4, float p_drop, uint64_t seed, int64_t drop_base, float* bias_partials, int n_partials,
                             void* hprev_out, const int* sum_idx, const void* dh_src, int zero_row,
                             const void* w_ih_t, void* dinp, int64_t ld_dinp, int n_in, int dinp_accumulate, float p_in, uint64_t seed_in,
-                            int64_t in_drop_base, void* stream);
+                            int64_t in_drop_base, void* stream, int zero_from);
 
 int gtos_gru_weight_grads(int rows, int hs, int in_dim, int in_valid, const void* d4, const void* x, int64_t ldx, const void* hprev, int64_t ldh,
                           float* dwih, int64_t ld_dwih, float* dwhh, int64_t ld_dwhh, void* workspace, int64_t workspace_bytes, void* stream);
```
